# PJLab-ADG/neuralsim

Hardware: NVIDIA H100
Metric: Mrays/sec fwd+bwd (higher is better)
Workload: dtype f16

## Files before the change

### neuralsim_b200/csrc/color_tc.cu

```cuda
#include "fused_tc_common.cuh"
#include "sh_device.cuh"

namespace nsb {

struct ColorNetDev {
    DecoderDevTC dec;
    const __half *R1, *rb1, *R2, *rb2, *R3, *rb3;
    int rw, rin, n_appear;
    float fac[3];
};

constexpr int XW = 64;
constexpr int kTileBytes = kTile * XW * 2;
constexpr int kChunk = kTile * 16;

__host__ __device__ inline int ref_col(int k, int n_appear) {
    if (k < 32) return 22 + k;
    if (k < 35) return k - 32;
    if (k < 51) return 3 + (k - 35);
    if (k < 54) return 19 + (k - 51);
    if (k < 54 + n_appear) return k;
    return -1;
}


__device__ __forceinline__ void level_jacobian(const PLMeta &m, uint32_t p, const float (&xs)[3], const __half *__restrict__ grid,
                                               float (&J0)[3], float (&J1)[3]) {
    uint32_t cell[8];
    float w[8], fr[3], scale[3];
    level_cells3(m, p, xs, cell, w, fr, scale);
    const uint32_t *lp = level_cells_ptr(m, p, grid);
    float2 v[8];
#pragma unroll
    for (int c = 0; c < 8; ++c) {
        const uint32_t raw = ld_nc_u32(lp + cell[c]);
        v[c] = __half22float2(*reinterpret_cast<const __half2 *>(&raw));
    }
#pragma unroll
    for (int gd = 0; gd < 3; ++gd) {
        float a0 = 0.f, a1 = 0.f;
#pragma unroll
        for (int c = 0; c < 4; ++c) {
            float ww = scale[gd];
            int left = 0;
#pragma unroll
            for (int k = 0; k < 2; ++k) {
                const int d = k >= gd ? k + 1 : k;
                if (c & (1 << k)) { ww = __fmul_rn(ww, fr[d]); left += 1 << d; }
                else ww = __fmul_rn(ww, __fsub_rn(1.f, fr[d]));
            }
            const int right = left + (1 << gd);
            a0 = __fmaf_rn(ww, __fsub_rn(v[right].x, v[left].x), a0);
            a1 = __fmaf_rn(ww, __fsub_rn(v[right].y, v[left].y), a1);
        }
        J0[gd] = a0;
        J1[gd] = a1;
    }
}

__device__ __forceinline__ void unpack8(const uint4 &q, float (&v)[8]) {
    const __half2 *h = reinterpret_cast<const __half2 *>(&q);
#pragma unroll
    for (int i = 0; i < 4; ++i) { const float2 f = __half22float2(h[i]); v[2 * i] = f.x; v[2 * i + 1] = f.y; }
}

constexpr int kColorGatherU = 4;

constexpr int kColorBwdCtasPerSM = 2;

__global__ void __launch_bounds__(kTile)
k_color_fwd(const PLMeta m, const __half *__restrict__ grid, const ColorNetDev net, const PointSrc ps, const float *__restrict__ view_dirs,
            const float *__restrict__ h_appear, int64_t n, int max_level, float *__restrict__ sdf_out, float *__restrict__ nab_out,
            float *__restrict__ rgb_out, float *__restrict__ x_out, uint8_t *__restrict__ Zt, uint8_t *__restrict__ Xt,
            uint8_t *__restrict__ Y1t, uint8_t *__restrict__ Y2t, const OccCollect oc, const int64_t *__restrict__ n_dev) {
    n = eff_n(n, n_dev);
    extern __shared__ uint8_t dyn_smem[];
    uint8_t *tiles = reinterpret_cast<uint8_t *>((reinterpret_cast<uintptr_t>(dyn_smem) + 1023) & ~uintptr_t(1023));
    uint8_t *sX = tiles;
    uint8_t *sU = sX + kTileBytes;
    uint8_t *sW1 = sU + kTileBytes;
    uint8_t *sW1T = sW1 + HW * NF * 2;
    uint8_t *sR1 = sW1T + HW * NF * 2;
    uint8_t *sR2 = sR1 + XW * XW * 2;
    constexpr int kS = tc::acc_stride(64);
    float *acc = reinterpret_cast<float *>(sR2 + XW * XW * 2);
    __shared__ float sb1[HW], sW2[HW], srb1[XW], srb2[XW], sR3[3][XW];
    __shared__ float sb2, srb3[3];

    const int tid = threadIdx.x;
    stage_W1(net.dec, sW1, tid);
    stage_W1T(net.dec, sW1T, tid);
    for (int e = tid; e < XW * XW; e += kTile) {
        const int j = e % XW, k = e / XW;
        const int rc = ref_col(k, net.n_appear);
        const __half v1 = (j < net.rw && rc >= 0) ? net.R1[j * net.rin + rc] : __float2half_rn(0.f);
        const __half v2 = (j < net.rw && k < net.rw) ? net.R2[j * net.rw + k] : __float2half_rn(0.f);
        *reinterpret_cast<__half *>(sR1 + (k / 8) * (XW * 16) + j * 16 + (k % 8) * 2) = v1;
        *reinterpret_cast<__half *>(sR2 + (k / 8) * (XW * 16) + j * 16 + (k % 8) * 2) = v2;
    }
    stage_decoder_vectors(net.dec, sb1, sW2, &sb2, tid);
    if (tid < XW) {
        srb1[tid] = tid < net.rw ? __half2float(net.rb1[tid]) : 0.f;
        srb2[tid] = tid < net.rw ? __half2float(net.rb2[tid]) : 0.f;
#pragma unroll
        for (int k = 0; k < 3; ++k) sR3[k][tid] = tid < net.rw ? __half2float(net.R3[k * net.rw + tid]) : 0.f;
    }
    if (tid == 0) {
        for (int k = 0; k < 3; ++k) srb3[k] = __half2float(net.rb3[k]);
    }
    tc::fence_async_smem();
    __syncthreads();
    const uint32_t x_addr = tc::smem_u32(sX), u_addr = tc::smem_u32(sU), w1_addr = tc::smem_u32(sW1), w1t_addr = tc::smem_u32(sW1T);
    const uint32_t r1_addr = tc::smem_u32(sR1), r2_addr = tc::smem_u32(sR2);
    const SoftplusK spk(net.dec.beta);

    const int64_t n_tiles = (n + kTile - 1) / kTile;
    for (int64_t tile = blockIdx.x; tile < n_tiles; tile += gridDim.x) {
        const int64_t i = tile * kTile + tid;
        const bool valid = i < n;
        float xn[3], xs[3];
        int64_t ray;
        load_point(ps, ps.x == nullptr, i, valid, xn, xs, ray);
        gather_row_to_tile<kTile, kColorGatherU>(m, grid, xs, max_level, sX, tid);
        tc::fence_async_smem();
        __syncthreads();
        tc::mma_to_rows<64, 0, 0, NF / 16>(acc, kS, 0, tc::kmajor(x_addr, kTile), tc::kmajor(w1_addr, HW), false);
        __syncthreads();
        float out = 0.f;
        uint8_t *zt = Zt ? Zt + tile * kTileBytes : nullptr;
#pragma unroll 1
        for (int c = 0; c < HW / 8; ++c) {
            float z[8], uu[8];
            tc::acc_ld8(acc, kS, tid, c * 8, z);
#pragma unroll
            for (int j = 0; j < 8; ++j) {
                z[j] = r16(z[j] + sb1[c * 8 + j]);
                float a, s;
                softplus_as(z[j], spk, a, s);
                out = fmaf(r16(a), sW2[c * 8 + j], out);
                uu[j] = sW2[c * 8 + j] * s;
            }
            *reinterpret_cast<uint4 *>(sU + c * kChunk + tid * 16) = tc::pack8_f16(uu);
            if (zt) *reinterpret_cast<uint4 *>(zt + c * kChunk + tid * 16) = tc::pack8_f16(z);
        }
        const float sdf = r16(out + sb2);
        tc::fence_async_smem();
        __syncthreads();
        tc::mma_to_rows<32, 0, 0, HW / 16>(acc, kS, 0, tc::kmajor(u_addr, kTile), tc::kmajor(w1t_addr, NF), false);
        __syncthreads();
        float nacc[3] = {0.f, 0.f, 0.f};
#pragma unroll 1
        for (uint32_t g4 = 0; g4 < 4; ++g4) {
            float gg[8];
            tc::acc_ld8(acc, kS, tid, g4 * 8, gg);
#pragma unroll
            for (uint32_t q = 0; q < 4; ++q) {
                const uint32_t p = g4 * 4 + q;
                if ((int)m.level[p] <= max_level) {
                    float J0[3], J1[3];
                    level_jacobian(m, p, xs, grid, J0, J1);
                    const float g0 = r16(gg[2 * q]), g1 = r16(gg[2 * q + 1]);
#pragma unroll
                    for (int d = 0; d < 3; ++d) nacc[d] = __fmaf_rn(g0, J0[d], nacc[d]);
#pragma unroll
                    for (int d = 0; d < 3; ++d) nacc[d] = __fmaf_rn(g1, J1[d], nacc[d]);
                }
            }
        }
        float nab[3];
#pragma unroll
        for (int d = 0; d < 3; ++d) nab[d] = __fmul_rn(__fmul_rn(nacc[d], 0.5f), net.fac[d]);
        {
            float xr[32];
#pragma unroll
            for (int k = 0; k < 32; ++k) xr[k] = 0.f;
            xr[0] = xn[0]; xr[1] = xn[1]; xr[2] = xn[2];
            if (valid) {
                sh_basis(view_dirs[ray * 3], view_dirs[ray * 3 + 1], view_dirs[ray * 3 + 2], 4, xr + 3);
                if (h_appear) {
#pragma unroll
                    for (int k = 0; k < 8; ++k)
                        if (k < net.n_appear) xr[22 + k] = h_appear[ray * net.n_appear + k];
                }
            }
#pragma unroll
            for (int d = 0; d < 3; ++d) xr[19 + d] = fminf(fmaxf(nab[d], -1.f), 1.f);
            uint8_t *xt = Xt ? Xt + tile * kTileBytes : nullptr;
#pragma unroll
            for (int c = 0; c < 4; ++c) {
                float v8[8];
#pragma unroll
                for (int k = 0; k < 8; ++k) v8[k] = xr[c * 8 + k];
                const uint4 q = tc::pack8_f16(v8);
                *reinterpret_cast<uint4 *>(sX + (4 + c) * kChunk + tid * 16) = q;
                if (xt) {
                    *reinterpret_cast<uint4 *>(xt + (4 + c) * kChunk + tid * 16) = q;
                    *reinterpret_cast<uint4 *>(xt + c * kChunk + tid * 16) = *reinterpret_cast<const uint4 *>(sX + c * kChunk + tid * 16);
                }
            }
        }
        tc::fence_async_smem();
        __syncthreads();
        tc::mma_to_rows<64, 0, 0, XW / 16>(acc, kS, 0, tc::kmajor(x_addr, kTile), tc::kmajor(r1_addr, XW), false);
        __syncthreads();
        uint8_t *y1t = Y1t ? Y1t + tile * kTileBytes : nullptr;
#pragma unroll 1
        for (int c = 0; c < XW / 8; ++c) {
            float y[8];
            tc::acc_ld8(acc, kS, tid, c * 8, y);
#pragma unroll
            for (int j = 0; j < 8; ++j) y[j] = fmaxf(r16(y[j] + srb1[c * 8 + j]), 0.f);
            const uint4 q = tc::pack8_f16(y);
            *reinterpret_cast<uint4 *>(sU + c * kChunk + tid * 16) = q;
            if (y1t) *reinterpret_cast<uint4 *>(y1t + c * kChunk + tid * 16) = q;
        }
        tc::fence_async_smem();
        __syncthreads();
        tc::mma_to_rows<64, 0, 0, XW / 16>(acc, kS, 0, tc::kmajor(u_addr, kTile), tc::kmajor(r2_addr, XW), false);
        __syncthreads();
        float o3[3] = {0.f, 0.f, 0.f};
        uint8_t *y2t = Y2t ? Y2t + tile * kTileBytes : nullptr;
#pragma unroll 1
        for (int c = 0; c < XW / 8; ++c) {
            float y[8];
            tc::acc_ld8(acc, kS, tid, c * 8, y);
#pragma unroll
            for (int j = 0; j < 8; ++j) {
                y[j] = fmaxf(r16(y[j] + srb2[c * 8 + j]), 0.f);
#pragma unroll
                for (int k = 0; k < 3; ++k) o3[k] = fmaf(y[j], sR3[k][c * 8 + j], o3[k]);
            }
            if (y2t) *reinterpret_cast<uint4 *>(y2t + c * kChunk + tid * 16) = tc::pack8_f16(y);
        }
        if (valid) {
            sdf_out[i] = sdf;
            if (oc.pcl) occ_collect_point(oc, xs, sdf);
#pragma unroll
            for (int d = 0; d < 3; ++d) {
                nab_out[i * 3 + d] = nab[d];
                const float y3 = r16(o3[d] + srb3[d]);
                rgb_out[i * 3 + d] = r16(1.f / (1.f + expf(-y3)));
                if (x_out) x_out[i * 3 + d] = xn[d];
            }
        }
        __syncthreads();
    }
}

__global__ void __launch_bounds__(kTile, kColorBwdCtasPerSM)
k_color_rad_bwd(const ColorNetDev net, const uint8_t *__restrict__ Xt, const uint8_t *__restrict__ Y1t, const uint8_t *__restrict__ Y2t,
                const float *__restrict__ rgb, const float *__restrict__ g_rgb, int64_t n, float *__restrict__ dh_out,
                float *__restrict__ dR1, float *__restrict__ drb1, float *__restrict__ dR2, float *__restrict__ drb2,
                float *__restrict__ dR3, float *__restrict__ drb3, const int64_t *__restrict__ n_dev) {
    n = eff_n(n, n_dev);
    constexpr int NE = 80;
    extern __shared__ uint8_t dyn_smem[];
    uint8_t *tiles = reinterpret_cast<uint8_t *>((reinterpret_cast<uintptr_t>(dyn_smem) + 1023) & ~uintptr_t(1023));
    uint8_t *sT = tiles;
    uint8_t *sY1 = sT + 3 * kTileBytes;
    uint8_t *sXe = sY1 + kTile * NE * 2;
    uint8_t *sR2T = sXe + kTile * NE * 2;
    uint8_t *sR1h = sR2T + XW * XW * 2;
    __shared__ float sR3[3][XW];
    __shared__ float sdb3[3];
    __shared__ __align__(8) uint64_t mbar_ld;

    const int tid = threadIdx.x, lane = tid & 31;
    for (int e = tid; e < XW * XW; e += kTile) {
        const int i = e % XW, j = e / XW;
        const __half v = (j < net.rw && i < net.rw) ? net.R2[j * net.rw + i] : __float2half_rn(0.f);
        *reinterpret_cast<__half *>(sR2T + (j / 8) * (XW * 16) + i * 16 + (j % 8) * 2) = v;
    }
    for (int e = tid; e < NF * XW; e += kTile) {
        const int k = e % NF, j = e / NF;
        const __half v = j < net.rw ? net.R1[j * net.rin + 22 + k] : __float2half_rn(0.f);
        *reinterpret_cast<__half *>(sR1h + (j / 8) * (NF * 16) + k * 16 + (j % 8) * 2) = v;
    }
    if (tid < XW) {
#pragma unroll
        for (int k = 0; k < 3; ++k) sR3[k][tid] = tid < net.rw ? __half2float(net.R3[k * net.rw + tid]) : 0.f;
    }
    *reinterpret_cast<uint4 *>(sY1 + 8 * kChunk + tid * 16) = make_uint4(0x00003C00u, 0, 0, 0);
    *reinterpret_cast<uint4 *>(sY1 + 9 * kChunk + tid * 16) = make_uint4(0, 0, 0, 0);
    *reinterpret_cast<uint4 *>(sXe + 9 * kChunk + tid * 16) = make_uint4(0, 0, 0, 0);
    float xa[NE / 2], xb[NE / 2], x3[4];
#pragma unroll
    for (int k = 0; k < NE / 2; ++k) xa[k] = xb[k] = 0.f;
#pragma unroll
    for (int k = 0; k < 4; ++k) x3[k] = 0.f;
    if (tid == 0) {
        sdb3[0] = sdb3[1] = sdb3[2] = 0.f;
        tc::mbar_init(&mbar_ld, 1);
        tc::fence_mbar_init();
    }
    tc::fence_async_smem();
    __syncthreads();
    const uint32_t t_addr = tc::smem_u32(sT), y1_addr = tc::smem_u32(sY1), xe_addr = tc::smem_u32(sXe);
    const uint32_t r2t_addr = tc::smem_u32(sR2T), r1h_addr = tc::smem_u32(sR1h);
    uint32_t ld_phase = 0;
    bool first_tile = true;

    const int64_t n_tiles = (n + kTile - 1) / kTile;
    auto fetch = [&](int64_t tile) {
        tc::mbar_arrive_expect_tx(&mbar_ld, 3 * kTileBytes);
        tc::tma_load_bulk(sT + 2 * kTileBytes, Y2t + tile * kTileBytes, kTileBytes, &mbar_ld);
        tc::tma_load_bulk(sY1, Y1t + tile * kTileBytes, kTileBytes, &mbar_ld);
        tc::tma_load_bulk(sXe, Xt + tile * kTileBytes, kTileBytes, &mbar_ld);
    };
    if (tid == 0 && (int64_t)blockIdx.x < n_tiles) fetch(blockIdx.x);
    for (int64_t tile = blockIdx.x; tile < n_tiles; tile += gridDim.x) {
        const int64_t i = tile * kTile + tid;
        const bool valid = i < n;
        tc::mbar_wait(&mbar_ld, ld_phase);
        ld_phase ^= 1;
        float gy[3] = {0.f, 0.f, 0.f};
        if (valid && g_rgb) {
#pragma unroll
            for (int k = 0; k < 3; ++k) {
                const float y = rgb[i * 3 + k];
                gy[k] = r16(r16(g_rgb[i * 3 + k]) * ((1.f - y) * y));
            }
        }
        {
            float e8[8] = {1.f, gy[0], gy[1], gy[2], 0.f, 0.f, 0.f, 0.f};
            *reinterpret_cast<uint4 *>(sXe + 8 * kChunk + tid * 16) = tc::pack8_f16(e8);
        }
#pragma unroll
        for (int k = 0; k < 3; ++k) {
            const float sgy = warp_sum(gy[k]);
            if (lane == 0 && sgy != 0.f) atomicAdd(&sdb3[k], sgy);
        }
#pragma unroll 1
        for (int c = 0; c < 8; ++c) {
            float y2[8], d[8];
            unpack8(*reinterpret_cast<const uint4 *>(sT + 2 * kTileBytes + c * kChunk + tid * 16), y2);
#pragma unroll
            for (int j = 0; j < 8; ++j) {
                const float v = gy[0] * sR3[0][c * 8 + j] + gy[1] * sR3[1][c * 8 + j] + gy[2] * sR3[2][c * 8 + j];
                d[j] = y2[j] > 0.f ? v : 0.f;
            }
            *reinterpret_cast<uint4 *>(sT + c * kChunk + tid * 16) = tc::pack8_f16(d);
        }
        tc::fence_async_smem();
        __syncthreads();
        {
            float dy[2][XW / 2];
            tc::mma_m128<64, 0, 0, XW / 16>(dy, tc::kmajor(t_addr, kTile), tc::kmajor(r2t_addr, XW), false);
#pragma unroll
            for (int h = 0; h < 2; ++h)
#pragma unroll
                for (int c = 0; c < XW / 8; ++c)
#pragma unroll
                    for (int r = 0; r < 2; ++r) {
                        const uint32_t off = tc::pair_off<kTile>(h * 64 + tc::frag_row(r), tc::frag_col(c));
                        const float2 y1 = tc::ld_pair_f16(sY1, off);
                        tc::st_pair_f16(sT + kTileBytes, off, y1.x > 0.f ? dy[h][4 * c + 2 * r] : 0.f, y1.y > 0.f ? dy[h][4 * c + 2 * r + 1] : 0.f);
                    }
        }
        tc::fence_async_smem();
        __syncthreads();
        float dh[2][NF / 2];
        tc::mma_m128<32, 0, 0, XW / 16>(dh, tc::kmajor(t_addr + kTileBytes, kTile), tc::kmajor(r1h_addr, NF), false);
        tc::mma_m64<NE, 1, 1, kTile / 16>(xa, tc::mnmajor(t_addr, kTile), tc::mnmajor(y1_addr, kTile), true);
        tc::mma_m64<NE, 1, 1, kTile / 16>(xb, tc::mnmajor(t_addr + kTileBytes, kTile), tc::mnmajor(xe_addr, kTile), true);
        tc::mma_m64<8, 1, 1, kTile / 16>(x3, tc::mnmajor(t_addr + 2 * kTileBytes, kTile), tc::mnmajor(xe_addr + 8 * kChunk, kTile), true);
        first_tile = false;
        __syncthreads();
        if (tid == 0 && tile + gridDim.x < n_tiles) {
            tc::fence_async_smem();
            fetch(tile + gridDim.x);
        }
#pragma unroll
        for (int h = 0; h < 2; ++h)
#pragma unroll
            for (int r = 0; r < 2; ++r) {
                const int64_t row = tile * kTile + h * 64 + tc::frag_row(r);
                if (row < n) {
#pragma unroll
                    for (int c = 0; c < NF / 8; ++c)
                        *reinterpret_cast<float2 *>(dh_out + row * NF + tc::frag_col(c)) = make_float2(dh[h][4 * c + 2 * r], dh[h][4 * c + 2 * r + 1]);
                }
            }
    }
    if (!first_tile) {
#pragma unroll
        for (int r = 0; r < 2; ++r) {
            const int row = tc::frag_row(r);
            if (row >= net.rw) continue;
#pragma unroll
            for (int c = 0; c < NE / 8; ++c)
#pragma unroll
                for (int j = 0; j < 2; ++j) {
                    const int col = tc::frag_col(c) + j;
                    const float a = xa[4 * c + 2 * r + j], b = xb[4 * c + 2 * r + j];
                    if (col < XW) {
                        if (col < net.rw) atomicAdd(dR2 + row * net.rw + col, a);
                        const int rc = ref_col(col, net.n_appear);
                        if (rc >= 0) atomicAdd(dR1 + row * net.rin + rc, b);
                    } else if (col == XW) {
                        atomicAdd(drb2 + row, a);
                        atomicAdd(drb1 + row, b);
                    }
                }
#pragma unroll
            for (int j = 0; j < 2; ++j) {
                const int col = tc::frag_col(0) + j;
                if (col >= 1 && col <= 3) atomicAdd(dR3 + (col - 1) * net.rw + row, x3[2 * r + j]);
            }
        }
        if (tid < 3) atomicAdd(drb3 + tid, sdb3[tid]);
    }
}

__global__ void __launch_bounds__(kTile, kColorBwdCtasPerSM)
k_color_sdf_bwd(const PLMeta m, const __half *__restrict__ grid, const ColorNetDev net, const PointSrc ps, const uint8_t *__restrict__ Zt,
                const uint8_t *__restrict__ Xt, const float *__restrict__ g_nab, const float *__restrict__ g_sdf, const float *__restrict__ dh_r,
                int64_t n, int max_level, float *__restrict__ d_grid, float *__restrict__ d_W1, float *__restrict__ d_b1, float *__restrict__ d_W2,
                float *__restrict__ d_b2, const int64_t *__restrict__ n_dev) {
    n = eff_n(n, n_dev);
    constexpr int NX = 48;
    extern __shared__ uint8_t dyn_smem[];
    uint8_t *tiles = reinterpret_cast<uint8_t *>((reinterpret_cast<uintptr_t>(dyn_smem) + 1023) & ~uintptr_t(1023));
    uint8_t *sT = tiles;
    uint8_t *sHe = sT + 3 * kTileBytes;
    uint8_t *sGe = sHe + kTile * NX * 2;
    uint8_t *sW1 = sGe + kTile * NX * 2;
    uint8_t *sW1T = sW1 + HW * NF * 2;
    uint8_t *sZ = sW1T + NF * HW * 2;
    constexpr int kS = tc::acc_stride(2 * NF);
    float *stage = reinterpret_cast<float *>(sT);
    static_assert(kTile * kS * 4 <= 3 * kTileBytes, "the staged rows must fit in T");
    __shared__ float sW2[HW], sdsdf[kTile];
    __shared__ float sdb2;
    __shared__ __align__(8) uint64_t mbar_ld;

    const int tid = threadIdx.x, lane = tid & 31;
    stage_W1(net.dec, sW1, tid);
    stage_W1T(net.dec, sW1T, tid);
    stage_decoder_vectors(net.dec, nullptr, sW2, nullptr, tid);
    *reinterpret_cast<uint4 *>(sHe + 4 * kChunk + tid * 16) = make_uint4(0x00003C00u, 0, 0, 0);
    *reinterpret_cast<uint4 *>(sGe + 4 * kChunk + tid * 16) = make_uint4(0x00003C00u, 0, 0, 0);
    *reinterpret_cast<uint4 *>(sHe + 5 * kChunk + tid * 16) = make_uint4(0, 0, 0, 0);
    *reinterpret_cast<uint4 *>(sGe + 5 * kChunk + tid * 16) = make_uint4(0, 0, 0, 0);
    float wacc[NX / 2], vacc[4];
#pragma unroll
    for (int k = 0; k < NX / 2; ++k) wacc[k] = 0.f;
#pragma unroll
    for (int k = 0; k < 4; ++k) vacc[k] = 0.f;
    if (tid == 0) {
        sdb2 = 0.f;
        tc::mbar_init(&mbar_ld, 1);
        tc::fence_mbar_init();
    }
    tc::fence_async_smem();
    __syncthreads();
    const uint32_t t_addr = tc::smem_u32(sT), he_addr = tc::smem_u32(sHe), ge_addr = tc::smem_u32(sGe), w1_addr = tc::smem_u32(sW1),
                   w1t_addr = tc::smem_u32(sW1T);
    const SoftplusK spk(net.dec.beta);
    uint32_t ld_phase = 0;
    bool first_tile = true;

    const int64_t n_tiles = (n + kTile - 1) / kTile;
    auto fetch = [&](int64_t tile) {
        tc::mbar_arrive_expect_tx(&mbar_ld, kTileBytes + 4 * kChunk);
        tc::tma_load_bulk(sZ, Zt + tile * kTileBytes, kTileBytes, &mbar_ld);
        tc::tma_load_bulk(sHe, Xt + tile * kTileBytes, 4 * kChunk, &mbar_ld);
    };
    if (tid == 0 && (int64_t)blockIdx.x < n_tiles) fetch(blockIdx.x);
    for (int64_t tile = blockIdx.x; tile < n_tiles; tile += gridDim.x) {
        const int64_t i = tile * kTile + tid;
        const bool valid = i < n;
        float xn[3], xs[3];
        int64_t ray;
        load_point(ps, ps.x == nullptr, i, valid, xn, xs, ray);
        float gin[3] = {0.f, 0.f, 0.f};
        if (valid && g_nab) {
#pragma unroll
            for (int d = 0; d < 3; ++d) gin[d] = g_nab[i * 3 + d] * net.fac[d] * 0.5f;
        }
        const float dsdf = (valid && g_sdf) ? g_sdf[i] : 0.f;
        sdsdf[tid] = dsdf;
        tc::mbar_wait(&mbar_ld, ld_phase);
        ld_phase ^= 1;
#pragma unroll 1
        for (int c = 0; c < 8; ++c) {
            float z[8], uu[8];
            unpack8(*reinterpret_cast<const uint4 *>(sZ + c * kChunk + tid * 16), z);
#pragma unroll
            for (int j = 0; j < 8; ++j) {
                float a, s;
                softplus_as(z[j], spk, a, s);
                uu[j] = sW2[c * 8 + j] * s;
            }
            *reinterpret_cast<uint4 *>(sT + kTileBytes + c * kChunk + tid * 16) = tc::pack8_f16(uu);
        }
#pragma unroll 4
        for (uint32_t p = 0; p < 16; ++p) {
            uint32_t packed = 0;
            if ((int)m.level[p] <= max_level) {
                float J0[3], J1[3];
                level_jacobian(m, p, xs, grid, J0, J1);
                float a0 = 0.f, a1 = 0.f;
#pragma unroll
                for (int d = 0; d < 3; ++d) { a0 = __fmaf_rn(gin[d], J0[d], a0); a1 = __fmaf_rn(gin[d], J1[d], a1); }
                const __half2 h = __floats2half2_rn(a0, a1);
                packed = *reinterpret_cast<const uint32_t *>(&h);
            }
            *reinterpret_cast<uint32_t *>(sGe + (p >> 2) * kChunk + tid * 16 + (p & 3) * 4) = packed;
        }
        tc::fence_async_smem();
        __syncthreads();
        float gfr[2][NF / 2];
        {
            float du[2][HW / 2];
            tc::mma_m128<64, 0, 0, NF / 16>(du, tc::kmajor(ge_addr, kTile), tc::kmajor(w1_addr, HW), false);
            tc::mma_m128<32, 0, 0, HW / 16>(gfr, tc::kmajor(t_addr + kTileBytes, kTile), tc::kmajor(w1t_addr, NF), false);
#pragma unroll
            for (int h = 0; h < 2; ++h)
#pragma unroll
                for (int r = 0; r < 2; ++r) {
                    const int row = h * 64 + tc::frag_row(r);
                    const float ds = sdsdf[row];
#pragma unroll
                    for (int c = 0; c < HW / 8; ++c) {
                        const int col = tc::frag_col(c);
                        const uint32_t off = tc::pair_off<kTile>(row, col);
                        const float2 z2 = tc::ld_pair_f16(sZ, off);
                        float dz[2], vv[2];
#pragma unroll
                        for (int j = 0; j < 2; ++j) {
                            const float z = j ? z2.y : z2.x;
                            float a, s;
                            softplus_as(z, spk, a, s);
                            const float w2 = sW2[col + j], d = r16(du[h][4 * c + 2 * r + j]);
                            const float curv = (z * spk.k > spk.thr) ? 0.f : spk.beta * s * (1.f - s);
                            dz[j] = d * w2 * curv + ds * w2 * s;
                            vv[j] = d * s + ds * r16(a);
                        }
                        tc::st_pair_f16(sT, off, dz[0], dz[1]);
                        tc::st_pair_f16(sT + 2 * kTileBytes, off, vv[0], vv[1]);
                    }
                }
        }
        tc::fence_async_smem();
        __syncthreads();
        float dhz[2][NF / 2];
        tc::mma_m128<32, 0, 0, HW / 16>(dhz, tc::kmajor(t_addr, kTile), tc::kmajor(w1t_addr, NF), false);
        tc::mma_m64<NX, 1, 1, kTile / 16>(wacc, tc::mnmajor(t_addr, kTile), tc::mnmajor(he_addr, kTile), true);
        tc::mma_m64<NF, 1, 1, kTile / 16>(*reinterpret_cast<float(*)[NF / 2]>(wacc), tc::mnmajor(t_addr + kTileBytes, kTile), tc::mnmajor(ge_addr, kTile), true);
        tc::mma_m64<8, 1, 1, kTile / 16>(vacc, tc::mnmajor(t_addr + 2 * kTileBytes, kTile), tc::mnmajor(ge_addr + 4 * kChunk, kTile), true);
        first_tile = false;
        const float dsum = warp_sum(dsdf);
        if (lane == 0 && dsum != 0.f) atomicAdd(&sdb2, dsum);
        __syncthreads();
        if (tid == 0 && tile + gridDim.x < n_tiles) {
            tc::fence_async_smem();
            fetch(tile + gridDim.x);
        }
        tc::frag_store<NF>(gfr, stage, kS, 0);
        tc::frag_store<NF>(dhz, stage, kS, NF);
        __syncthreads();
#pragma unroll 1
        for (uint32_t g4 = 0; g4 < 4; ++g4) {
            float gg[8], hz[8];
            tc::acc_ld8(stage, kS, tid, g4 * 8, gg);
            tc::acc_ld8(stage, kS, tid, NF + g4 * 8, hz);
            if (valid && dh_r) {
                const float4 r0 = *reinterpret_cast<const float4 *>(dh_r + i * NF + g4 * 8), r1 = *reinterpret_cast<const float4 *>(dh_r + i * NF + g4 * 8 + 4);
                hz[0] += r0.x; hz[1] += r0.y; hz[2] += r0.z; hz[3] += r0.w; hz[4] += r1.x; hz[5] += r1.y; hz[6] += r1.z; hz[7] += r1.w;
            }
#pragma unroll
            for (uint32_t q = 0; q < 4; ++q) {
                const uint32_t p = g4 * 4 + q;
                if ((int)m.level[p] > max_level) continue;
                uint32_t cell[8];
                float w[8], fr[3], sc[3], ua[8], ub[8];
                level_cells3(m, p, xs, cell, w, fr, sc);
                const float g0 = valid ? r16(gg[2 * q]) : 0.f, g1 = valid ? r16(gg[2 * q + 1]) : 0.f;
                const float h0 = valid ? hz[2 * q] : 0.f, h1 = valid ? hz[2 * q + 1] : 0.f;
#pragma unroll
                for (int c = 0; c < 8; ++c) {
                    float wsum = 0.f;
#pragma unroll
                    for (int gd = 0; gd < 3; ++gd) {
                        float ww = __fmul_rn(sc[gd], gin[gd]);
#pragma unroll
                        for (int d = 0; d < 3; ++d) {
                            if (d == gd) continue;
                            ww = __fmul_rn(ww, (c & (1 << d)) ? fr[d] : __fsub_rn(1.f, fr[d]));
                        }
                        wsum += (c & (1 << gd)) ? ww : -ww;
                    }
                    ua[c] = g0 * wsum + h0 * w[c];
                    ub[c] = g1 * wsum + h1 * w[c];
                }
                bool issue = valid;
                if (level_mergeable(m, p)) issue = warp_merge_updates(cell_key3(m, p, xs), valid, ua, ub, lane);
                if (issue) {
                    float2 *gp = level_grad_ptr(m, p, d_grid);
#pragma unroll
                    for (int c = 0; c < 8; ++c) red_add2(gp + cell[c], ua[c], ub[c]);
                }
            }
        }
        __syncthreads();
    }
    if (!first_tile) {
#pragma unroll
        for (int r = 0; r < 2; ++r) {
            const int row = tc::frag_row(r);
            if (row >= net.dec.width) continue;
#pragma unroll
            for (int c = 0; c <= NF / 8; ++c)
#pragma unroll
                for (int j = 0; j < 2; ++j) {
                    const int col = tc::frag_col(c) + j;
                    if (col < NF) atomicAdd(d_W1 + row * NF + col, wacc[4 * c + 2 * r + j]);
                    else if (col == NF) atomicAdd(d_b1 + row, wacc[4 * c + 2 * r + j]);
                }
            if (tc::frag_col(0) == 0) atomicAdd(d_W2 + row, vacc[2 * r]);
        }
        if (tid == 0) atomicAdd(d_b2, sdb2);
    }
}

}

using namespace nsb;

namespace {
int make_net(const nsb_color_net *c, const nsb_lotd_meta *meta, PLMeta *m, ColorNetDev *d, const char *who) {
    const nsb_sdf_decoder dec{c->W1, c->b1, c->W2, c->b2, c->width, c->beta};
    if (int rc = make_decoder(meta, &dec, m, &d->dec, who)) return rc;
    NSB_REQUIRE(c->rad_width >= 1 && c->rad_width <= 64, "%s: radiance width must be <= 64", who);
    NSB_REQUIRE(c->n_appear >= 0 && c->n_appear <= 8 && c->rad_in == 54 + c->n_appear,
                "%s: radiance input must be [x(3), SH deg 4 (16), n(3), h(32), h_appear(<=8)]", who);
    d->R1 = (const __half *)c->R1; d->rb1 = (const __half *)c->rb1; d->R2 = (const __half *)c->R2; d->rb2 = (const __half *)c->rb2;
    d->R3 = (const __half *)c->R3; d->rb3 = (const __half *)c->rb3;
    d->rw = c->rad_width; d->rin = c->rad_in; d->n_appear = c->n_appear;
    for (int k = 0; k < 3; ++k) d->fac[k] = c->nablas_scale[k];
    return 0;
}
}

static int64_t n_tiles(int64_t n) { return (n + kTile - 1) / kTile; }

extern "C" int64_t nsb_color_tile_bytes(int64_t n) { return n_tiles(n) * (int64_t)kTileBytes; }

extern "C" int nsb_fused_color_fwd(const nsb_lotd_meta *meta, const void *params_half, const nsb_color_net *net, const float *x, const float *rays_o,
                                   const float *rays_d, const int64_t *ridx, const float *t, const float *view_dirs, const float *h_appear,
                                   int64_t n, int32_t max_level, float *sdf, float *nablas, float *rgb, float *x_out, void *act_z, void *act_x,
                                   void *act_y1, void *act_y2, const nsb_occ_collect *collect, void *stream) {
    const DevCounts dn = take_counts();
    if (n == 0) return 0;
    NSB_REQUIRE(meta && params_half && net && sdf && nablas && rgb && view_dirs, "nsb_fused_color_fwd: NULL argument");
    NSB_REQUIRE(x || (rays_o && rays_d && t), "nsb_fused_color_fwd: need x or (rays_o, rays_d, t)");
    NSB_REQUIRE((act_z && act_x && act_y1 && act_y2) || (!act_z && !act_x && !act_y1 && !act_y2), "nsb_fused_color_fwd: pass all four activation buffers or none");
    PLMeta m;
    ColorNetDev d;
    if (int rc = make_net(net, meta, &m, &d, "nsb_fused_color_fwd")) return rc;
    NSB_REQUIRE(d.n_appear == 0 || h_appear, "nsb_fused_color_fwd: h_appear is NULL but the net has %d appearance channels", d.n_appear);
    constexpr int kSmem = 2 * kTileBytes + 2 * HW * NF * 2 + 2 * XW * XW * 2 + kTile * tc::acc_stride(64) * 4 + 1024;
    opt_in_smem(k_color_fwd, kSmem);
    const PointSrc ps{x, rays_o, rays_d, t, ridx};
    k_color_fwd<<<persistent_grid(n_tiles(n), 2), kTile, kSmem, (cudaStream_t)stream>>>(m, (const __half *)params_half, d, ps, view_dirs, h_appear, n,
                                                                                        max_level < 0 ? -1 : max_level, sdf, nablas, rgb, x_out, (uint8_t *)act_z,
                                                                                        (uint8_t *)act_x, (uint8_t *)act_y1, (uint8_t *)act_y2,
                                                                                        occ_collect_of(collect), dn.a);
    return check_launch("nsb_fused_color_fwd");
}

extern "C" int nsb_fused_color_bwd(const nsb_lotd_meta *meta, const void *params_half, const nsb_color_net *net, const float *x, const float *rays_o,
                                   const float *rays_d, const int64_t *ridx, const float *t, int64_t n, int32_t max_level, const void *act_z,
                                   const void *act_x, const void *act_y1, const void *act_y2, const float *rgb, const float *g_sdf,
                                   const float *g_nablas, const float *g_rgb, float *dh_scratch, float *d_grid, float *d_W1, float *d_b1,
                                   float *d_W2, float *d_b2, float *d_R1, float *d_rb1, float *d_R2, float *d_rb2, float *d_R3, float *d_rb3,
                                   void *stream) {
    const DevCounts dn = take_counts();
    if (n == 0) return 0;
    NSB_REQUIRE(meta && params_half && net && act_z && act_x && act_y1 && act_y2 && rgb && dh_scratch, "nsb_fused_color_bwd: NULL argument");
    NSB_REQUIRE(d_grid && d_W1 && d_b1 && d_W2 && d_b2 && d_R1 && d_rb1 && d_R2 && d_rb2 && d_R3 && d_rb3, "nsb_fused_color_bwd: NULL gradient buffer");
    NSB_REQUIRE(x || (rays_o && rays_d && t), "nsb_fused_color_bwd: need x or (rays_o, rays_d, t)");
    PLMeta m;
    ColorNetDev d;
    if (int rc = make_net(net, meta, &m, &d, "nsb_fused_color_bwd")) return rc;
    cudaStream_t s = (cudaStream_t)stream;
    const float *dh = nullptr;
    if (g_rgb) {
        constexpr int kSmemR = 3 * kTileBytes + 2 * kTile * 80 * 2 + XW * XW * 2 + NF * XW * 2 + 1024;
        opt_in_smem(k_color_rad_bwd, kSmemR);
        if (int rc = require_ctas_per_sm(k_color_rad_bwd, kTile, kSmemR, kColorBwdCtasPerSM, "nsb_fused_color_bwd(radiance)")) return rc;
        k_color_rad_bwd<<<persistent_grid(n_tiles(n), kColorBwdCtasPerSM), kTile, kSmemR, s>>>(d, (const uint8_t *)act_x, (const uint8_t *)act_y1,
                                                                                               (const uint8_t *)act_y2, rgb, g_rgb, n, dh_scratch, d_R1,
                                                                                               d_rb1, d_R2, d_rb2, d_R3, d_rb3, dn.a);
        if (int rc = check_launch("nsb_fused_color_bwd(radiance)")) return rc;
        dh = dh_scratch;
    }
    constexpr int kSmemS = 3 * kTileBytes + 2 * kTile * 48 * 2 + 2 * HW * NF * 2 + kTileBytes + 1024;
    opt_in_smem(k_color_sdf_bwd, kSmemS);
    if (int rc = require_ctas_per_sm(k_color_sdf_bwd, kTile, kSmemS, kColorBwdCtasPerSM, "nsb_fused_color_bwd(sdf)")) return rc;
    const PointSrc ps{x, rays_o, rays_d, t, ridx};
    k_color_sdf_bwd<<<persistent_grid(n_tiles(n), kColorBwdCtasPerSM), kTile, kSmemS, s>>>(m, (const __half *)params_half, d, ps, (const uint8_t *)act_z, (const uint8_t *)act_x,
                                                                          g_nablas, g_sdf, dh, n, max_level < 0 ? -1 : max_level, d_grid, d_W1, d_b1, d_W2, d_b2, dn.a);
    return check_launch("nsb_fused_color_bwd(sdf)");
}
```

### neuralsim_b200/csrc/tc_util.cuh

```cuda
#pragma once
#include "nsb_common.cuh"

namespace nsb {
namespace tc {

__device__ __forceinline__ uint32_t smem_u32(const void *p) { return (uint32_t)__cvta_generic_to_shared(p); }

__device__ __forceinline__ uint64_t make_desc(uint32_t smem_addr, uint32_t lbo_bytes, uint32_t sbo_bytes) {
    uint64_t d = 0;
    d |= (uint64_t)((smem_addr >> 4) & 0x3FFF);
    d |= (uint64_t)((lbo_bytes >> 4) & 0x3FFF) << 16;
    d |= (uint64_t)((sbo_bytes >> 4) & 0x3FFF) << 32;
    return d;
}

struct Operand {
    uint32_t addr, lbo, sbo, kstep;
};
__device__ __forceinline__ Operand kmajor(uint32_t addr, int rows) { return Operand{addr, (uint32_t)rows * 16, 128, (uint32_t)rows * 32}; }
__device__ __forceinline__ Operand mnmajor(uint32_t addr, int rows) { return Operand{addr, 128, (uint32_t)rows * 16, 256}; }

template <int N, int TA, int TB>
struct Wgmma;
template <int TA, int TB>
struct Wgmma<8, TA, TB> {
    __device__ __forceinline__ static void mma(float (&d)[4], uint64_t a, uint64_t b, uint32_t acc) {
        asm volatile(
            "{\n\t.reg .pred p;\n\tsetp.ne.b32 p, %6, 0;\n\t"
            "wgmma.mma_async.sync.aligned.m64n8k16.f32.f16.f16 {%0, %1, %2, %3}, %4, %5, p, 1, 1, %7, %8;\n\t}\n"
            : "+f"(d[0]), "+f"(d[1]), "+f"(d[2]), "+f"(d[3])
            : "l"(a), "l"(b), "r"(acc), "n"(TA), "n"(TB));
    }
};
template <int TA, int TB>
struct Wgmma<32, TA, TB> {
    __device__ __forceinline__ static void mma(float (&d)[16], uint64_t a, uint64_t b, uint32_t acc) {
        asm volatile(
            "{\n\t.reg .pred p;\n\tsetp.ne.b32 p, %18, 0;\n\t"
            "wgmma.mma_async.sync.aligned.m64n32k16.f32.f16.f16 {%0, %1, %2, %3, %4, %5, %6, %7, %8, %9, %10, %11, %12, %13, %14, %15}, %16, %17, p, 1, 1, %19, %20;\n\t}\n"
            : "+f"(d[0]), "+f"(d[1]), "+f"(d[2]), "+f"(d[3]), "+f"(d[4]), "+f"(d[5]), "+f"(d[6]), "+f"(d[7]), "+f"(d[8]), "+f"(d[9]), "+f"(d[10]), "+f"(d[11]), "+f"(d[12]), "+f"(d[13]), "+f"(d[14]), "+f"(d[15])
            : "l"(a), "l"(b), "r"(acc), "n"(TA), "n"(TB));
    }
};
template <int TA, int TB>
struct Wgmma<40, TA, TB> {
    __device__ __forceinline__ static void mma(float (&d)[20], uint64_t a, uint64_t b, uint32_t acc) {
        asm volatile(
            "{\n\t.reg .pred p;\n\tsetp.ne.b32 p, %22, 0;\n\t"
            "wgmma.mma_async.sync.aligned.m64n40k16.f32.f16.f16 {%0, %1, %2, %3, %4, %5, %6, %7, %8, %9, %10, %11, %12, %13, %14, %15, %16, %17, %18, %19}, %20, %21, p, 1, 1, %23, %24;\n\t}\n"
            : "+f"(d[0]), "+f"(d[1]), "+f"(d[2]), "+f"(d[3]), "+f"(d[4]), "+f"(d[5]), "+f"(d[6]), "+f"(d[7]), "+f"(d[8]), "+f"(d[9]), "+f"(d[10]), "+f"(d[11]), "+f"(d[12]), "+f"(d[13]), "+f"(d[14]), "+f"(d[15]), "+f"(d[16]), "+f"(d[17]), "+f"(d[18]), "+f"(d[19])
            : "l"(a), "l"(b), "r"(acc), "n"(TA), "n"(TB));
    }
};
template <int TA, int TB>
struct Wgmma<48, TA, TB> {
    __device__ __forceinline__ static void mma(float (&d)[24], uint64_t a, uint64_t b, uint32_t acc) {
        asm volatile(
            "{\n\t.reg .pred p;\n\tsetp.ne.b32 p, %26, 0;\n\t"
            "wgmma.mma_async.sync.aligned.m64n48k16.f32.f16.f16 {%0, %1, %2, %3, %4, %5, %6, %7, %8, %9, %10, %11, %12, %13, %14, %15, %16, %17, %18, %19, %20, %21, %22, %23}, %24, %25, p, 1, 1, %27, %28;\n\t}\n"
            : "+f"(d[0]), "+f"(d[1]), "+f"(d[2]), "+f"(d[3]), "+f"(d[4]), "+f"(d[5]), "+f"(d[6]), "+f"(d[7]), "+f"(d[8]), "+f"(d[9]), "+f"(d[10]), "+f"(d[11]), "+f"(d[12]), "+f"(d[13]), "+f"(d[14]), "+f"(d[15]), "+f"(d[16]), "+f"(d[17]), "+f"(d[18]), "+f"(d[19]), "+f"(d[20]), "+f"(d[21]), "+f"(d[22]), "+f"(d[23])
            : "l"(a), "l"(b), "r"(acc), "n"(TA), "n"(TB));
    }
};
template <int TA, int TB>
struct Wgmma<64, TA, TB> {
    __device__ __forceinline__ static void mma(float (&d)[32], uint64_t a, uint64_t b, uint32_t acc) {
        asm volatile(
            "{\n\t.reg .pred p;\n\tsetp.ne.b32 p, %34, 0;\n\t"
            "wgmma.mma_async.sync.aligned.m64n64k16.f32.f16.f16 {%0, %1, %2, %3, %4, %5, %6, %7, %8, %9, %10, %11, %12, %13, %14, %15, %16, %17, %18, %19, %20, %21, %22, %23, %24, %25, %26, %27, %28, %29, %30, %31}, %32, %33, p, 1, 1, %35, %36;\n\t}\n"
            : "+f"(d[0]), "+f"(d[1]), "+f"(d[2]), "+f"(d[3]), "+f"(d[4]), "+f"(d[5]), "+f"(d[6]), "+f"(d[7]), "+f"(d[8]), "+f"(d[9]), "+f"(d[10]), "+f"(d[11]), "+f"(d[12]), "+f"(d[13]), "+f"(d[14]), "+f"(d[15]), "+f"(d[16]), "+f"(d[17]), "+f"(d[18]), "+f"(d[19]), "+f"(d[20]), "+f"(d[21]), "+f"(d[22]), "+f"(d[23]), "+f"(d[24]), "+f"(d[25]), "+f"(d[26]), "+f"(d[27]), "+f"(d[28]), "+f"(d[29]), "+f"(d[30]), "+f"(d[31])
            : "l"(a), "l"(b), "r"(acc), "n"(TA), "n"(TB));
    }
};
template <int TA, int TB>
struct Wgmma<80, TA, TB> {
    __device__ __forceinline__ static void mma(float (&d)[40], uint64_t a, uint64_t b, uint32_t acc) {
        asm volatile(
            "{\n\t.reg .pred p;\n\tsetp.ne.b32 p, %42, 0;\n\t"
            "wgmma.mma_async.sync.aligned.m64n80k16.f32.f16.f16 {%0, %1, %2, %3, %4, %5, %6, %7, %8, %9, %10, %11, %12, %13, %14, %15, %16, %17, %18, %19, %20, %21, %22, %23, %24, %25, %26, %27, %28, %29, %30, %31, %32, %33, %34, %35, %36, %37, %38, %39}, %40, %41, p, 1, 1, %43, %44;\n\t}\n"
            : "+f"(d[0]), "+f"(d[1]), "+f"(d[2]), "+f"(d[3]), "+f"(d[4]), "+f"(d[5]), "+f"(d[6]), "+f"(d[7]), "+f"(d[8]), "+f"(d[9]), "+f"(d[10]), "+f"(d[11]), "+f"(d[12]), "+f"(d[13]), "+f"(d[14]), "+f"(d[15]), "+f"(d[16]), "+f"(d[17]), "+f"(d[18]), "+f"(d[19]), "+f"(d[20]), "+f"(d[21]), "+f"(d[22]), "+f"(d[23]), "+f"(d[24]), "+f"(d[25]), "+f"(d[26]), "+f"(d[27]), "+f"(d[28]), "+f"(d[29]), "+f"(d[30]), "+f"(d[31]), "+f"(d[32]), "+f"(d[33]), "+f"(d[34]), "+f"(d[35]), "+f"(d[36]), "+f"(d[37]), "+f"(d[38]), "+f"(d[39])
            : "l"(a), "l"(b), "r"(acc), "n"(TA), "n"(TB));
    }
};

__device__ __forceinline__ void wgmma_fence() { asm volatile("wgmma.fence.sync.aligned;" ::: "memory"); }
__device__ __forceinline__ void wgmma_commit() { asm volatile("wgmma.commit_group.sync.aligned;" ::: "memory"); }
__device__ __forceinline__ void wgmma_wait_all() { asm volatile("wgmma.wait_group.sync.aligned 0;" ::: "memory"); }
__device__ __forceinline__ void fence_operand(float &r) { asm volatile("" : "+f"(r)::"memory"); }

template <int N, int TA, int TB, int KSTEPS>
__device__ __forceinline__ void mma_m128(float (&d)[2][N / 2], const Operand &a, const Operand &b, bool accumulate) {
#pragma unroll
    for (int h = 0; h < 2; ++h)
#pragma unroll
        for (int i = 0; i < N / 2; ++i) fence_operand(d[h][i]);
    wgmma_fence();
#pragma unroll
    for (int h = 0; h < 2; ++h)
#pragma unroll
        for (int ks = 0; ks < KSTEPS; ++ks)
            Wgmma<N, TA, TB>::mma(d[h], make_desc(a.addr + h * 8 * a.sbo + ks * a.kstep, a.lbo, a.sbo), make_desc(b.addr + ks * b.kstep, b.lbo, b.sbo),
                                  (ks > 0 || accumulate) ? 1u : 0u);
    wgmma_commit();
    wgmma_wait_all();
#pragma unroll
    for (int h = 0; h < 2; ++h)
#pragma unroll
        for (int i = 0; i < N / 2; ++i) fence_operand(d[h][i]);
}

template <int N, int TA, int TB, int KSTEPS>
__device__ __forceinline__ void mma_m64(float (&d)[N / 2], const Operand &a, const Operand &b, bool accumulate) {
#pragma unroll
    for (int i = 0; i < N / 2; ++i) fence_operand(d[i]);
    wgmma_fence();
#pragma unroll
    for (int ks = 0; ks < KSTEPS; ++ks)
        Wgmma<N, TA, TB>::mma(d, make_desc(a.addr + ks * a.kstep, a.lbo, a.sbo), make_desc(b.addr + ks * b.kstep, b.lbo, b.sbo),
                              (ks > 0 || accumulate) ? 1u : 0u);
    wgmma_commit();
    wgmma_wait_all();
#pragma unroll
    for (int i = 0; i < N / 2; ++i) fence_operand(d[i]);
}

__device__ __forceinline__ int frag_row(int i) { return (threadIdx.x >> 5) * 16 + ((threadIdx.x & 31) >> 2) + 8 * i; }
__device__ __forceinline__ int frag_col(int c) { return c * 8 + 2 * (threadIdx.x & 3); }
template <int R>
__device__ __forceinline__ uint32_t pair_off(int row, int col) { return (uint32_t)((col >> 3) * (R * 16) + row * 16 + (col & 7) * 2); }
__device__ __forceinline__ float2 ld_pair_f16(const uint8_t *tile, uint32_t off) {
    return __half22float2(*reinterpret_cast<const __half2 *>(tile + off));
}
__device__ __forceinline__ void st_pair_f16(uint8_t *tile, uint32_t off, float a, float b) {
    *reinterpret_cast<__half2 *>(tile + off) = __floats2half2_rn(a, b);
}

constexpr int acc_stride(int cols) { return cols + 4; }

template <int N>
__device__ __forceinline__ void frag_store(const float (&d)[2][N / 2], float *acc, int stride, int col0) {
    const int w = threadIdx.x >> 5, l = threadIdx.x & 31;
#pragma unroll
    for (int h = 0; h < 2; ++h)
#pragma unroll
        for (int c = 0; c < N / 8; ++c)
#pragma unroll
            for (int i = 0; i < 2; ++i) {
                const int row = h * 64 + w * 16 + (l >> 2) + 8 * i, col = col0 + c * 8 + 2 * (l & 3);
                *reinterpret_cast<float2 *>(acc + row * stride + col) = make_float2(d[h][4 * c + 2 * i], d[h][4 * c + 2 * i + 1]);
            }
}
template <int N>
__device__ __forceinline__ void frag_load(float (&d)[2][N / 2], const float *acc, int stride, int col0) {
    const int w = threadIdx.x >> 5, l = threadIdx.x & 31;
#pragma unroll
    for (int h = 0; h < 2; ++h)
#pragma unroll
        for (int c = 0; c < N / 8; ++c)
#pragma unroll
            for (int i = 0; i < 2; ++i) {
                const int row = h * 64 + w * 16 + (l >> 2) + 8 * i, col = col0 + c * 8 + 2 * (l & 3);
                const float2 v = *reinterpret_cast<const float2 *>(acc + row * stride + col);
                d[h][4 * c + 2 * i] = v.x;
                d[h][4 * c + 2 * i + 1] = v.y;
            }
}
template <int N, int TA, int TB, int KSTEPS>
__device__ __forceinline__ void mma_to_rows(float *acc, int stride, int col0, const Operand &a, const Operand &b, bool accumulate) {
    float d[2][N / 2];
    if (accumulate) frag_load<N>(d, acc, stride, col0);
    else {
#pragma unroll
        for (int h = 0; h < 2; ++h)
#pragma unroll
            for (int i = 0; i < N / 2; ++i) d[h][i] = 0.f;
    }
    mma_m128<N, TA, TB, KSTEPS>(d, a, b, accumulate);
    frag_store<N>(d, acc, stride, col0);
}

__device__ __forceinline__ void acc_ld8(const float *acc, int stride, int row, int col, float (&v)[8]) {
    const float4 a = *reinterpret_cast<const float4 *>(acc + row * stride + col), b = *reinterpret_cast<const float4 *>(acc + row * stride + col + 4);
    v[0] = a.x; v[1] = a.y; v[2] = a.z; v[3] = a.w; v[4] = b.x; v[5] = b.y; v[6] = b.z; v[7] = b.w;
}

__device__ __forceinline__ void mbar_init(uint64_t *bar, uint32_t count) {
    asm volatile("mbarrier.init.shared::cta.b64 [%0], %1;" ::"r"(smem_u32(bar)), "r"(count) : "memory");
}
__device__ __forceinline__ void mbar_wait(uint64_t *bar, uint32_t parity) {
    asm volatile(
        "{\n\t.reg .pred p;\n\tWAIT_%=:\n\t"
        "mbarrier.try_wait.parity.shared::cta.b64 p, [%0], %1;\n\t"
        "@p bra DONE_%=;\n\tbra WAIT_%=;\n\tDONE_%=:\n\t}\n" ::"r"(smem_u32(bar)),
        "r"(parity)
        : "memory");
}

__device__ __forceinline__ void mbar_arrive_expect_tx(uint64_t *bar, uint32_t bytes) {
    asm volatile("mbarrier.arrive.expect_tx.shared::cta.b64 _, [%0], %1;" ::"r"(smem_u32(bar)), "r"(bytes) : "memory");
}
__device__ __forceinline__ void tma_load_bulk(void *smem_dst, const void *gmem_src, uint32_t bytes, uint64_t *bar) {
    asm volatile("cp.async.bulk.shared::cluster.global.mbarrier::complete_tx::bytes [%0], [%1], %2, [%3];" ::"r"(smem_u32(smem_dst)), "l"(gmem_src),
                 "r"(bytes), "r"(smem_u32(bar))
                 : "memory");
}

__device__ __forceinline__ void fence_async_smem() { asm volatile("fence.proxy.async.shared::cta;" ::: "memory"); }
__device__ __forceinline__ void fence_mbar_init() { asm volatile("fence.mbarrier_init.release.cluster;" ::: "memory"); }

__device__ __forceinline__ uint4 pack8_f16(const float (&v)[8]) {
    __half2 h0 = __floats2half2_rn(v[0], v[1]), h1 = __floats2half2_rn(v[2], v[3]);
    __half2 h2 = __floats2half2_rn(v[4], v[5]), h3 = __floats2half2_rn(v[6], v[7]);
    uint4 q;
    q.x = *reinterpret_cast<uint32_t *>(&h0); q.y = *reinterpret_cast<uint32_t *>(&h1);
    q.z = *reinterpret_cast<uint32_t *>(&h2); q.w = *reinterpret_cast<uint32_t *>(&h3);
    return q;
}

template <int R, int K>
__device__ __forceinline__ void store_row_f16(uint8_t *tile, int r, const float *vals) {
#pragma unroll
    for (int c = 0; c < K / 8; ++c) {
        __half2 h0 = __floats2half2_rn(vals[c * 8 + 0], vals[c * 8 + 1]);
        __half2 h1 = __floats2half2_rn(vals[c * 8 + 2], vals[c * 8 + 3]);
        __half2 h2 = __floats2half2_rn(vals[c * 8 + 4], vals[c * 8 + 5]);
        __half2 h3 = __floats2half2_rn(vals[c * 8 + 6], vals[c * 8 + 7]);
        uint4 q;
        q.x = *reinterpret_cast<uint32_t *>(&h0);
        q.y = *reinterpret_cast<uint32_t *>(&h1);
        q.z = *reinterpret_cast<uint32_t *>(&h2);
        q.w = *reinterpret_cast<uint32_t *>(&h3);
        *reinterpret_cast<uint4 *>(tile + c * (R * 16) + r * 16) = q;
    }
}

}
}
```

### neuralsim_b200/fields/fused_color.py

```python
from __future__ import annotations

import ctypes

import torch
from torch import autograd

from .. import _lib as L


class _FusedColor(autograd.Function):
    @staticmethod
    def forward(ctx, model, pts, view_dirs, h_appear, max_level, keep, collect, *params):
        grid16, net, _held = model._fused_color_state()
        ridx, t, rays_o, rays_d = pts
        n, dev = t.numel(), t.device
        meta = model.implicit_surface.encoding.meta
        sdf = torch.empty(n, dtype=torch.float32, device=dev)
        nab = torch.empty(n, 3, dtype=torch.float32, device=dev)
        rgb = torch.empty(n, 3, dtype=torch.float32, device=dev)
        x = torch.empty(n, 3, dtype=torch.float32, device=dev)
        acts = None
        if keep:
            acts = torch.empty(4, int(L.lib().nsb_color_tile_bytes(L.c_i64(n))), dtype=torch.uint8, device=dev)
        ap = [L.ptr(acts[k]) if keep else None for k in range(4)]
        with L.KERNEL_TIMER.time("fused_color_fwd", n):
            L.check(L.lib().nsb_fused_color_fwd(meta.c_ref, L.ptr(grid16, "f16"), ctypes.byref(net), None, L.ptr(rays_o, "f32"), L.ptr(rays_d, "f32"),
                                                L.ptr(ridx, "i64"), L.ptr(t, "f32"), L.ptr(view_dirs, "f32"), L.ptr(h_appear, "f32", allow_none=True),
                                                L.c_i64(n), L.c_i32(max_level), L.ptr(sdf), L.ptr(nab), L.ptr(rgb), L.ptr(x), *ap,
                                                ctypes.byref(collect) if collect is not None else None, L.stream_ptr()),
                    "fused_color_fwd")
        ctx.model, ctx.pts, ctx.max_level, ctx.n = model, pts, max_level, n
        ctx.held = (grid16, net, _held, acts, rgb)
        ctx.shapes = [p.shape for p in params]
        ctx.set_materialize_grads(False)
        ctx.mark_non_differentiable(x)
        return sdf, nab, rgb, x

    @staticmethod
    @autograd.function.once_differentiable
    def backward(ctx, g_sdf, g_nab, g_rgb, _gx):
        grid16, net, _held, acts, rgb = ctx.held
        if acts is None:
            raise RuntimeError("fused_color: backward through a forward that ran without grad")
        dev, n = rgb.device, ctx.n
        meta = ctx.model.implicit_surface.encoding.meta
        sizes = [int(torch.Size(s).numel()) for s in ctx.shapes[1:]]
        small = torch.zeros(sum(sizes), dtype=torch.float32, device=dev)
        grads, o = [torch.zeros(ctx.shapes[0], dtype=torch.float32, device=dev)], 0
        for sh, k in zip(ctx.shapes[1:], sizes):
            grads.append(small[o:o + k].view(sh))
            o += k
        if g_sdf is None and g_nab is None and g_rgb is None:
            return (None,) * 7 + tuple(grads)
        ridx, t, rays_o, rays_d = ctx.pts
        c = lambda g: None if g is None else g.contiguous().float()
        g_sdf, g_nab, g_rgb = c(g_sdf), c(g_nab), c(g_rgb)
        dh = torch.empty(n, 32, dtype=torch.float32, device=dev)
        with L.KERNEL_TIMER.time("fused_color_bwd", n):
            L.check(L.lib().nsb_fused_color_bwd(meta.c_ref, L.ptr(grid16, "f16"), ctypes.byref(net), None, L.ptr(rays_o, "f32"), L.ptr(rays_d, "f32"),
                                                L.ptr(ridx, "i64"), L.ptr(t, "f32"), L.c_i64(n), L.c_i32(ctx.max_level), L.ptr(acts[0]), L.ptr(acts[1]),
                                                L.ptr(acts[2]), L.ptr(acts[3]), L.ptr(rgb), L.ptr(g_sdf, allow_none=True), L.ptr(g_nab, allow_none=True),
                                                L.ptr(g_rgb, allow_none=True), L.ptr(dh), *[L.ptr(g) for g in grads], L.stream_ptr()),
                    "fused_color_bwd")
        return (None,) * 7 + tuple(grads)


def fused_color(model, ridx, t, rays_o, rays_d, view_dirs, h_appear=None, *, nablas_has_grad=True, collect=None):
    s, r = model.implicit_surface, model.radiance_net.blocks.layers
    d = s.decoder.layers
    params = (s.encoding.flattened_params, d[0].weight, d[0].bias, d[1].weight, d[1].bias, r[0].weight, r[0].bias, r[1].weight, r[1].bias,
              r[2].weight, r[2].bias)
    pts = (ridx.reshape(-1).contiguous().long(), t.detach().reshape(-1).contiguous().float(), rays_o.detach().contiguous().float(),
           rays_d.detach().contiguous().float())
    keep = torch.is_grad_enabled() and any(p.requires_grad for p in params)
    ha = None if h_appear is None else h_appear.detach().contiguous().float()
    sdf, nab, rgb, x = _FusedColor.apply(model, pts, view_dirs.detach().contiguous().float(), ha, s._ml(model.max_level), keep, collect, *params)
    if not nablas_has_grad:
        nab = nab.detach()
    return dict(sdf=sdf, nablas=nab, rgb=rgb, x=x)
```

### neuralsim_b200/graphics/neus_static.py

```python
from __future__ import annotations

import ctypes

import torch
import torch.nn.functional as F

from .. import _lib as L
from .raysample import batch_sample_step_linear
from .pack_ops import get_pack_infos_from_batch
from . import neus_fused as NF

__all__ = ["render_static", "StaticFrame", "CNT_SLOTS"]

CNT_SLOTS = dict(n_rays=0, pairs=2, marched_raw=3, hit_raw=4, kept_raw=6, kept_rays_raw=7, nonzero=9, marched=12, hit=13, fine0=14,
                 boundary=18, kept=19, overflow=20, kept_rays=21, merged0=22, rays_if_kept_fits=26)
_NULL = ctypes.c_void_p(0)
MARCH_ONEPASS = "auto"
MARCH_ONEPASS_MAX_BYTES = 64 << 20


def march_onepass(n_rays, max_steps):
    if MARCH_ONEPASS == "0":
        return False
    return MARCH_ONEPASS == "1" or 4 * int(n_rays) * int(max_steps) <= MARCH_ONEPASS_MAX_BYTES


def _slot(cnt, k):
    return ctypes.c_void_p(cnt.data_ptr() + 8 * k)


def _call(fn, what, cnt, k0, k1, *args):
    lib = L.lib()
    lib.nsb_bind_device_counts(_slot(cnt, k0), _slot(cnt, k1) if k1 is not None else _NULL)
    try:
        rc = fn(*args)
    finally:
        lib.nsb_bind_device_counts(_NULL, _NULL)
    L.check(rc, what)


def _scan(counts, cnt, slot, *, first=None, info2=None, index=None, pack=None, src=None, nz_src=None, ws=None):
    if ws is None:
        ws = torch.zeros(NF._scan_ws_bytes(), dtype=torch.uint8, device=counts.device)
    P = L.ptr
    L.check(L.lib().nsb_scan_counts(P(counts, "i32"), L.c_i64(counts.shape[0]), P(first, allow_none=True), P(info2, allow_none=True),
                                    P(index, allow_none=True), P(pack, allow_none=True), P(src, "i64", allow_none=True), P(nz_src, allow_none=True),
                                    _slot(cnt, slot), None, L.c_i64(0), P(ws), L.stream_ptr()), "scan_counts")


def _query_counts(cnt, phase, n_coarse1, num_fine, march_cap, kept_cap):
    nf = (ctypes.c_int32 * max(len(num_fine), 1))(*[int(n) for n in num_fine])
    L.check(L.lib().nsb_query_counts(ctypes.c_void_p(cnt.data_ptr()), L.c_i32(phase), L.c_i32(n_coarse1), nf, L.c_i32(len(num_fine)),
                                     L.c_i64(march_cap), L.c_i64(kept_cap), L.stream_ptr()), "query_counts")


def _sdf_launch(meta, grid16, dec, rays_o, rays_d, t, sdf, *, ridx=None, packs=None, ml, collect, cnt, slot, timer="lotd_gather"):
    P = L.ptr
    mode = 2 if packs is not None else 1
    with L.KERNEL_TIMER.time(timer, t.numel()):
        _call(L.lib().nsb_fused_sdf_collect, "fused_sdf", cnt, slot, None,
              meta.c_ref, P(grid16, "f16"), ctypes.byref(dec), None, P(rays_o, "f32"), P(rays_d, "f32"),
              P(ridx, "i64") if mode == 1 else None, P(t, "f32"), L.c_i64(t.numel()),
              P(packs[0], "i64") if mode == 2 else None, P(packs[1], "i64", allow_none=True) if mode == 2 else None,
              L.c_i64(packs[0].shape[0] if mode == 2 else 0), L.c_i32(mode), L.c_i32(ml), P(sdf),
              ctypes.byref(collect) if collect is not None else None, L.stream_ptr())
    return sdf


class _StaticSDF(torch.autograd.Function):

    @staticmethod
    def forward(ctx, st, ridx, t, packs, count_slot, grid, W1, b1, W2, b2):
        sdf = torch.empty(t.numel(), dtype=torch.float32, device=t.device)
        _sdf_launch(st.meta, st.grid16, st.dec, st.rays_o, st.rays_d, t, sdf, ridx=ridx if packs is None else None, packs=packs, ml=st.ml,
                    collect=st.collect, cnt=st.cnt, slot=count_slot, timer="fused_sdf_fwd")
        ctx.st, ctx.ridx, ctx.t = st, ridx, t
        ctx.shapes = (grid.shape, W1.shape, b1.shape, W2.shape, b2.shape)
        return sdf

    @staticmethod
    @torch.autograd.function.once_differentiable
    def backward(ctx, d_sdf):
        st, dev = ctx.st, d_sdf.device
        gs, w1s, b1s, w2s, b2s = ctx.shapes
        d_grid = torch.zeros(gs, dtype=torch.float32, device=dev)
        ks = [int(torch.Size(x).numel()) for x in (w1s, b1s, w2s, b2s)]
        small = torch.zeros(sum(ks), dtype=torch.float32, device=dev)
        d_W1, d_b1 = small[:ks[0]].view(w1s), small[ks[0]:ks[0] + ks[1]].view(b1s)
        d_W2, d_b2 = small[ks[0] + ks[1]:ks[0] + ks[1] + ks[2]].view(w2s), small[ks[0] + ks[1] + ks[2]:].view(b2s)
        d_sdf = d_sdf.contiguous().float()
        n = d_sdf.numel()
        P, cnt = L.ptr, st.cnt
        flag = torch.empty(n, dtype=torch.int32, device=dev)
        _call(L.lib().nsb_flag_nonzero, "flag_nonzero", cnt, CNT_SLOTS["boundary"], None, P(d_sdf, "f32"), L.c_i64(n), P(flag), L.stream_ptr())
        keep = torch.empty(n, dtype=torch.int64, device=dev)
        _scan(flag, cnt, CNT_SLOTS["nonzero"], index=keep, ws=st.ws[3])
        with L.KERNEL_TIMER.time("fused_sdf_bwd", n):
            _call(L.lib().nsb_fused_sdf_bwd_indexed, "fused_sdf_bwd", cnt, CNT_SLOTS["nonzero"], None,
                  st.meta.c_ref, P(st.grid16, "f16"), ctypes.byref(st.dec), None, P(st.rays_o, "f32"), P(st.rays_d, "f32"), P(ctx.ridx, "i64"),
                  P(ctx.t, "f32"), P(d_sdf, "f32"), P(keep, "i64"), L.c_i64(n), L.c_i32(st.ml), P(d_grid), P(d_W1), P(d_b1), P(d_W2), P(d_b2),
                  L.stream_ptr())
        return None, None, None, None, None, d_grid, d_W1, d_b1, d_W2, d_b2


class _StaticAlpha(torch.autograd.Function):

    @staticmethod
    def forward(ctx, sdf, inv_s, pack_infos, cnt, early_stop_eps, alpha_thre):
        sdf_c, inv_c = sdf.detach().contiguous().float(), inv_s.detach().contiguous().float().reshape(1)
        Pn, dev = pack_infos.shape[0], sdf_c.device
        alpha = torch.empty_like(sdf_c)
        sel = torch.empty(sdf_c.shape[0], dtype=torch.bool, device=dev)
        steps = torch.empty(Pn, dtype=torch.int32, device=dev)
        P = L.ptr
        _call(L.lib().nsb_neus_alpha_forward, "neus_alpha_forward", cnt, CNT_SLOTS["n_rays"], None, P(sdf_c, "f32"), P(pack_infos, "i64"), L.c_i64(Pn),
              P(inv_c, "f32"), L.c_f32(early_stop_eps), L.c_f32(alpha_thre), P(alpha), P(sel), P(steps), L.stream_ptr())
        ctx.save_for_backward(sdf_c, inv_c, pack_infos)
        ctx.cnt, ctx.inv_shape = cnt, inv_s.shape
        ctx.mark_non_differentiable(sel, steps)
        return alpha, sel, steps

    @staticmethod
    def backward(ctx, g_alpha, _gs, _gn):
        sdf_c, inv_c, pack_infos = ctx.saved_tensors
        g = g_alpha.contiguous().float()
        d_sdf = torch.empty_like(sdf_c)
        d_inv = torch.zeros(1, device=sdf_c.device, dtype=torch.float32)
        P = L.ptr
        _call(L.lib().nsb_neus_alpha_backward, "neus_alpha_backward", ctx.cnt, CNT_SLOTS["n_rays"], None, P(sdf_c, "f32"), P(pack_infos, "i64"),
              L.c_i64(pack_infos.shape[0]), P(inv_c, "f32"), P(g, "f32"), P(d_sdf), P(d_inv), L.stream_ptr())
        return (d_sdf if ctx.needs_input_grad[0] else None, d_inv.reshape(ctx.inv_shape) if ctx.needs_input_grad[1] else None, None, None, None, None)


class _StaticGather(torch.autograd.Function):

    @staticmethod
    def forward(ctx, src, pidx, gathered, cnt):
        ctx.save_for_backward(pidx)
        ctx.n, ctx.cnt = src.shape[0], cnt
        return gathered

    @staticmethod
    def backward(ctx, g):
        pidx, = ctx.saved_tensors
        g = g.contiguous().float()
        d = torch.zeros(ctx.n, dtype=torch.float32, device=g.device)
        P = L.ptr
        _call(L.lib().nsb_scatter_f32, "scatter_f32", ctx.cnt, CNT_SLOTS["kept"], None, P(g, "f32"), P(pidx, "i64"), L.c_i64(pidx.shape[0]), P(d), L.stream_ptr())
        return d, None, None, None


class _StaticColor(torch.autograd.Function):

    @staticmethod
    def forward(ctx, st, ridx, t, view_dirs, h_appear, keep_acts, *params):
        n, dev = t.numel(), t.device
        sdf = torch.empty(n, dtype=torch.float32, device=dev)
        nab = torch.empty(n, 3, dtype=torch.float32, device=dev)
        rgb = torch.empty(n, 3, dtype=torch.float32, device=dev)
        x = torch.empty(n, 3, dtype=torch.float32, device=dev)
        acts = torch.empty(4, int(L.lib().nsb_color_tile_bytes(L.c_i64(n))), dtype=torch.uint8, device=dev) if keep_acts else None
        ap = [L.ptr(acts[k]) if keep_acts else None for k in range(4)]
        P = L.ptr
        with L.KERNEL_TIMER.time("fused_color_fwd", n):
            _call(L.lib().nsb_fused_color_fwd, "fused_color_fwd", st.cnt, CNT_SLOTS["kept"], None,
                  st.meta.c_ref, P(st.grid16, "f16"), ctypes.byref(st.net), None, P(st.rays_o, "f32"), P(st.rays_d, "f32"), P(ridx, "i64"), P(t, "f32"),
                  P(view_dirs, "f32"), P(h_appear, "f32", allow_none=True), L.c_i64(n), L.c_i32(st.ml), P(sdf), P(nab), P(rgb), P(x), *ap,
                  ctypes.byref(st.collect) if st.collect is not None else None, L.stream_ptr())
        ctx.st, ctx.ridx, ctx.t, ctx.n = st, ridx, t, n
        ctx.held = (acts, rgb)
        ctx.shapes = [p.shape for p in params]
        ctx.set_materialize_grads(False)
        ctx.mark_non_differentiable(x)
        return sdf, nab, rgb, x

    @staticmethod
    @torch.autograd.function.once_differentiable
    def backward(ctx, g_sdf, g_nab, g_rgb, _gx):
        acts, rgb = ctx.held
        if acts is None:
            raise RuntimeError("static colour query: backward through a forward that ran without grad")
        st, dev, n = ctx.st, rgb.device, ctx.n
        sizes = [int(torch.Size(s).numel()) for s in ctx.shapes[1:]]
        small = torch.zeros(sum(sizes), dtype=torch.float32, device=dev)
        grads, o = [torch.zeros(ctx.shapes[0], dtype=torch.float32, device=dev)], 0
        for sh, k in zip(ctx.shapes[1:], sizes):
            grads.append(small[o:o + k].view(sh))
            o += k
        if g_sdf is None and g_nab is None and g_rgb is None:
            return (None,) * 6 + tuple(grads)
        c = lambda g: None if g is None else g.contiguous().float()
        g_sdf, g_nab, g_rgb = c(g_sdf), c(g_nab), c(g_rgb)
        dh = torch.empty(n, 32, dtype=torch.float32, device=dev)
        P = L.ptr
        with L.KERNEL_TIMER.time("fused_color_bwd", n):
            _call(L.lib().nsb_fused_color_bwd, "fused_color_bwd", st.cnt, CNT_SLOTS["kept"], None,
                  st.meta.c_ref, P(st.grid16, "f16"), ctypes.byref(st.net), None, P(st.rays_o, "f32"), P(st.rays_d, "f32"), P(ctx.ridx, "i64"),
                  P(ctx.t, "f32"), L.c_i64(n), L.c_i32(st.ml), P(acts[0]), P(acts[1]), P(acts[2]), P(acts[3]), P(rgb), P(g_sdf, allow_none=True),
                  P(g_nab, allow_none=True), P(g_rgb, allow_none=True), P(dh), *[P(g) for g in grads], L.stream_ptr())
        return (None,) * 6 + tuple(grads)


class _StaticComposite(torch.autograd.Function):

    @staticmethod
    def forward(ctx, alpha, t, rgb, nablas, pack_infos, ray_index, n_rays, cnt, normalize_depth, early_stop_eps, alpha_thre):
        a, tt = alpha.detach().contiguous().float(), t.detach().contiguous().float()
        r = None if rgb is None else rgb.detach().contiguous().float()
        nb = None if nablas is None else nablas.detach().contiguous().float()
        Pn, dev = pack_infos.shape[0], a.device
        vw = torch.empty_like(a)
        cols = 2 + (3 if r is not None else 0) + (3 if nb is not None else 0)
        buf = torch.zeros(cols * n_rays, device=dev)
        mask, depth = buf[:n_rays], buf[n_rays:2 * n_rays]
        rgb_o = buf[2 * n_rays:5 * n_rays].view(n_rays, 3) if r is not None else None
        o3 = 5 * n_rays if r is not None else 2 * n_rays
        nab_o = buf[o3:o3 + 3 * n_rays].view(n_rays, 3) if nb is not None else None
        P = L.ptr
        _call(L.lib().nsb_composite_forward, "composite_forward", cnt, CNT_SLOTS["kept_rays"], None, P(a, "f32"), P(tt, "f32"), P(r, "f32", allow_none=True),
              P(nb, "f32", allow_none=True), P(pack_infos, "i64"), L.c_i64(Pn), L.c_f32(early_stop_eps), L.c_f32(alpha_thre),
              ctypes.c_int(1 if normalize_depth else 0), P(ray_index, "i64"), P(vw), P(mask), P(depth), P(rgb_o, allow_none=True),
              P(nab_o, allow_none=True), L.stream_ptr())
        ctx.save_for_backward(a, tt, r, nb, vw, pack_infos, mask, depth, ray_index)
        ctx.cfg = (normalize_depth, early_stop_eps, alpha_thre, cnt)
        ctx.set_materialize_grads(False)
        empty = a.new_empty(0)
        return vw, mask, depth, (rgb_o if rgb_o is not None else empty), (nab_o if nab_o is not None else empty)

    @staticmethod
    def backward(ctx, g_vw, g_mask, g_depth, g_rgb, g_nab):
        a, tt, r, nb, vw, pack_infos, mask, depth, ray_index = ctx.saved_tensors
        normalize_depth, eps, thre, cnt = ctx.cfg

        def opt(g, present=True):
            return None if (g is None or not present) else g.contiguous().float()
        g_vw, g_mask, g_depth = opt(g_vw), opt(g_mask), opt(g_depth)
        g_rgb, g_nab = opt(g_rgb, r is not None), opt(g_nab, nb is not None)
        d_alpha = torch.empty_like(a)
        d_rgb = torch.empty_like(r) if r is not None else None
        d_nab = torch.empty_like(nb) if nb is not None else None
        P = L.ptr
        _call(L.lib().nsb_composite_backward, "composite_backward", cnt, CNT_SLOTS["kept_rays"], None,
              P(a, "f32"), P(tt, "f32"), P(r, allow_none=True), P(nb, allow_none=True), P(vw, "f32"), P(pack_infos, "i64"), L.c_i64(pack_infos.shape[0]),
              L.c_f32(eps), L.c_f32(thre), ctypes.c_int(1 if normalize_depth else 0), P(mask), P(depth), P(g_mask, allow_none=True),
              P(g_depth, allow_none=True), P(g_rgb, allow_none=True), P(g_nab, allow_none=True), P(g_vw, allow_none=True), P(ray_index, "i64"),
              P(d_alpha), P(d_rgb, allow_none=True), P(d_nab, allow_none=True), L.stream_ptr())
        return (d_alpha, None, d_rgb, d_nab) + (None,) * 7


class _State:
    __slots__ = ("meta", "grid16", "dec", "net", "held", "rays_o", "rays_d", "ml", "collect", "cnt", "ws")


def _fp16_images(model):
    s, b = model.implicit_surface, model.radiance_net.blocks.layers
    d = s.decoder.layers
    ps = [s.encoding.flattened_params, d[0].weight, d[0].bias, d[1].weight, d[1].bias, b[0].weight, b[0].bias, b[1].weight, b[1].bias, b[2].weight, b[2].bias]
    t = [torch.empty(p.shape, dtype=torch.half, device=p.device) for p in ps]
    with torch.no_grad():
        t[0].copy_(ps[0].detach())
        torch._foreach_copy_(t[1:], [p.detach() for p in ps[1:]])
    dec = L.SdfDecoderC(t[1].data_ptr(), t[2].data_ptr(), t[3].data_ptr(), t[4].data_ptr(), d[0].out_features, float(d[0].activation.beta))
    r3 = s.radius3d_original
    fk = (r3.data_ptr(), r3._version, float(s.sdf_scale))
    if getattr(model, "_fac_cache", (None,))[0] != fk:
        model._fac_cache = (fk, (s.sdf_scale / r3).float().tolist())
    net = L.ColorNetC(*[x.data_ptr() for x in t[1:]], d[0].out_features, b[0].out_features, b[0].in_features, b[0].in_features - 54,
                      float(d[0].activation.beta), (ctypes.c_float * 3)(*model._fac_cache[1]))
    return t, dec, net, ps


def static_supported(model, cfg):
    qp = dict(model.ray_query_cfg.get("query_param", {}) or {})
    occ = getattr(getattr(model, "accel", None), "occ", None)
    return (getattr(model, "_color_fusable", lambda: False)() and model.use_view_dirs and occ is not None and occ.occ_grid.dim() == 3
            and occ.occ_grid.numel() * 4 // 32 <= 96 * 1024 and qp.get("num_coarse", 0) > 0 and len(qp.get("upsample_inv_s_factors", (1, 4, 16))) <= 4
            and qp.get("coarse_step_cfg", {}).get("step_mode", "linear") == "linear" and (cfg.get("with_rgb", True) or cfg.get("with_normal", True)))


def render_static(model, rays_o, rays_d, rays_h_appear=None, *, near=None, far=None, march_cap, kept_cap, coherent=False, with_rgb=True, with_normal=True,
                  perturb=False, training=None, depth_use_normalized_vw=True, cnt=None):
    P, lib = L.ptr, L.lib()
    if perturb:
        raise RuntimeError("render_static: perturb=True is not built (random streams of capacity-sized draws differ from the reference's); "
                           "use the host-sized path (SingleVolumeRenderer.render)")
    training = model.training if training is None else training
    R, dev = rays_o.shape[0], rays_o.device
    qp = dict(model.ray_query_cfg.get("query_param", {}) or {})
    nc1 = int(qp["num_coarse"]) + 1
    factors = list(qp.get("upsample_inv_s_factors", (1, 4, 16)))
    n_stage = len(factors)
    num_fine = qp.get("num_fine", 8)
    num_fine = [num_fine] * n_stage if isinstance(num_fine, int) else list(num_fine)
    num_fine = [n // 2 * 2 + 1 for n in num_fine]
    nf_tot = int(sum(num_fine))
    upsample_inv_s = qp.get("upsample_inv_s", 64.) / model.upsample_s_divisor
    use_est = bool(qp.get("upsample_use_estimate_alpha", False))
    nablas_has_grad = bool(qp.get("nablas_has_grad", False))
    mc = dict(qp.get("march_cfg", {}))
    fac = mc.pop("step_size_factor", 1.0)
    step_size, dt_gamma = mc.get("step_size", 1e-3) * fac, mc.get("dt_gamma", 0.0) * fac
    max_steps, max_step_size = int(mc.get("max_steps", 512)), mc.get("max_step_size", 1e10)
    march_cap, kept_cap = int(march_cap), int(kept_cap)
    S_cap = R * (nc1 + nf_tot)
    if cnt is None:
        cnt = torch.zeros(32, dtype=torch.int64, device=dev)
    else:
        cnt.zero_()
    st = _State()
    st.cnt = cnt
    wsb = (NF._scan_ws_bytes() + 255) // 256 * 256
    st.ws = torch.zeros(4, wsb, dtype=torch.uint8, device=dev)
    with torch.no_grad():
        t16, st.dec, st.net, masters = _fp16_images(model)
        st.held, st.grid16 = t16, t16[0]
        st.meta = model.implicit_surface.encoding.meta
        st.ml = model.implicit_surface._ml(model.max_level)
        st.collect = model.accel.occ.collect_struct() if training else None
        sp = model.space
        if getattr(sp, "_host_cr", None) is None or sp._host_cr[0] != (sp.aabb.data_ptr(), sp.aabb._version):
            c, r = sp.center.tolist(), sp.radius3d.tolist()
            sp._host_cr = ((sp.aabb.data_ptr(), sp.aabb._version), (ctypes.c_float * 3)(*c), (ctypes.c_float * 3)(*r))
        o_n, d_n = torch.empty(R, 3, device=dev), torch.empty(R, 3, device=dev)
        nr, fr = torch.empty(R, device=dev), torch.empty(R, device=dev)
        flag = torch.empty(R, dtype=torch.int32, device=dev)
        L.check(lib.nsb_ray_test_aabb(P(rays_o.contiguous(), "f32"), P(rays_d.contiguous(), "f32"), L.c_i64(R), sp._host_cr[1], sp._host_cr[2],
                                      ctypes.c_int(0 if near is None else 1), L.c_f32(0. if near is None else near),
                                      ctypes.c_int(0 if far is None else 1), L.c_f32(0. if far is None else far), P(o_n), P(d_n), P(nr), P(fr), P(flag),
                                      _slot(cnt, CNT_SLOTS["pairs"]), L.stream_ptr()), "ray_test_aabb")
        rays_inds = torch.empty(R, dtype=torch.int64, device=dev)
        _scan(flag, cnt, CNT_SLOTS["n_rays"], index=rays_inds, ws=st.ws[0])
        ha = rays_h_appear.detach().contiguous().float() if (rays_h_appear is not None and model.use_h_appear) else None
        if ha is None and model.use_h_appear:
            ha = torch.zeros(R, model.radiance_net.blocks.layers[0].in_features - 54, device=dev)
        n_ha = ha.shape[1] if ha is not None else 0
        rbuf = torch.zeros(R * (8 + n_ha), device=dev)
        o_c, d_c = rbuf[:3 * R].view(R, 3), rbuf[3 * R:6 * R].view(R, 3)
        n_c, f_c = rbuf[6 * R:7 * R], rbuf[7 * R:8 * R]
        ha_c = rbuf[8 * R:].view(R, n_ha) if ha is not None else None
        _call(lib.nsb_gather_rays, "gather_rays", cnt, CNT_SLOTS["n_rays"], None, P(rays_inds, "i64"), L.c_i64(R), P(o_n), P(d_n), P(nr), P(fr), P(o_c), P(d_c),
              P(n_c), P(f_c), P(ha, allow_none=True), P(ha_c, allow_none=True), L.c_i32(0 if ha is None else ha.shape[1]), L.stream_ptr())
        st.rays_o, st.rays_d = o_c, d_c
        view_dirs = (d_c / d_c.norm(dim=-1).clamp_min(1.0e-10).unsqueeze(-1)).contiguous()
        coarse = batch_sample_step_linear(n_c, f_c, nc1, prefix_shape=[R], perturb=perturb).contiguous()
        occ_grid = model.accel.occ.occ_grid
        res = occ_grid.shape[-3:]
        g8 = occ_grid.contiguous().view(torch.uint8)
        bits = torch.empty((occ_grid.numel() + 31) // 32, dtype=torch.int32, device=dev)
        L.check(lib.nsb_pack_occ_bits(P(g8, "u8"), L.c_i64(occ_grid.numel()), P(bits), L.stream_ptr()), "pack_occ_bits")
        roi = torch.tensor([-1, -1, -1, 1, 1, 1], dtype=torch.float32, device=dev) if getattr(model, "_static_roi", None) is None else model._static_roi
        model._static_roi = roi
        margs = (L.c_i64(R), P(o_c, "f32"), P(d_c, "f32"), P(n_c, "f32"), P(f_c, "f32"), P(roi, "f32"), None, L.c_i32(res[0]), L.c_i32(res[1]), L.c_i32(res[2]),
                 P(g8, "u8"), L.c_f32(step_size), L.c_f32(max_step_size), L.c_f32(dt_gamma), ctypes.c_uint32(max_steps))
        num_steps = torch.empty(R, dtype=torch.int32, device=dev)
        rec_t = torch.empty(R * max_steps, dtype=torch.float32, device=dev) if march_onepass(R, max_steps) else None
        with L.KERNEL_TIMER.time("march", R):
            if rec_t is not None:
                _call(lib.nsb_ray_marching_record, "ray_marching_record", cnt, CNT_SLOTS["n_rays"], None, L.c_i64(R), P(o_c, "f32"), P(d_c, "f32"), P(n_c, "f32"),
                      P(f_c, "f32"), P(roi, "f32"), L.c_i32(res[0]), L.c_i32(res[1]), L.c_i32(res[2]), P(g8, "u8"), L.c_f32(step_size), L.c_f32(max_step_size),
                      L.c_f32(dt_gamma), ctypes.c_uint32(max_steps), P(num_steps), P(rec_t), P(bits), L.stream_ptr())
            else:
                _call(lib.nsb_ray_marching_listed, "ray_marching", cnt, CNT_SLOTS["n_rays"], None, *margs, None, P(num_steps), None, None, None, None, None, None,
                      L.c_i64(0), P(bits), L.stream_ptr())
        info2 = torch.empty(R, 2, dtype=torch.int32, device=dev)
        ridx_hit = torch.empty(R, dtype=torch.int64, device=dev)
        pack_infos = torch.empty(R, 2, dtype=torch.int64, device=dev)
        _scan(num_steps, cnt, CNT_SLOTS["marched_raw"], info2=info2, index=ridx_hit, pack=pack_infos, ws=st.ws[1])
        _query_counts(cnt, 0, nc1, num_fine, march_cap, kept_cap)
        depth = torch.empty(march_cap, dtype=torch.float32, device=dev)
        ridx32 = torch.empty(march_cap, dtype=torch.int32, device=dev)
        with L.KERNEL_TIMER.time("march", R):
            if rec_t is not None:
                _call(lib.nsb_march_compact, "march_compact", cnt, CNT_SLOTS["hit"], None, P(rec_t, "f32"), ctypes.c_uint32(max_steps), P(info2, "i32"),
                      P(ridx_hit, "i64"), L.c_i64(R), P(depth), P(ridx32), L.stream_ptr())
            else:
                _call(lib.nsb_ray_marching_listed, "ray_marching", cnt, CNT_SLOTS["hit"], None, *margs, P(info2), None, P(depth), None, P(ridx32), None, None,
                      P(ridx_hit, "i64"), L.c_i64(R), P(bits), L.stream_ptr())
        ridx = ridx32.long()
        from . import neus as GN
        fine_stages = None
        if GN.use_persistent_upsample(R):
            fine_all, _ovf = NF.upsample_rays(st.meta, st.grid16, st.dec, ridx_hit, pack_infos, depth, o_c, d_c, [upsample_inv_s * f for f in factors], num_fine,
                                              max_level=st.ml, max_steps=max_steps, use_estimate_alpha=use_est, collect=st.collect, count=(cnt, CNT_SLOTS["hit"]))
            factors_loop = []
        else:
            factors_loop = factors
        sdf = torch.empty(march_cap if factors_loop else 1, dtype=torch.float32, device=dev)
        if factors_loop:
            fine_stages = []
            _sdf_launch(st.meta, st.grid16, st.dec, o_c, d_c, depth, sdf, ridx=ridx, ml=st.ml, collect=st.collect, cnt=cnt, slot=CNT_SLOTS["marched"])
        for i, factor in enumerate(factors_loop):
            cdf = torch.empty(march_cap, dtype=torch.float32, device=dev)
            _call(lib.nsb_neus_upsample_cdf, "neus_upsample_cdf", cnt, CNT_SLOTS["hit"], None, P(sdf, "f32"), P(depth, "f32"), P(pack_infos, "i64"), L.c_i64(R),
                  L.c_f32(upsample_inv_s * factor), ctypes.c_int(1 if use_est else 0), L.c_f32(1e-4), L.c_f32(0.0), P(cdf), L.stream_ptr())
            nf = num_fine[i]
            fine = torch.empty(R, nf, dtype=torch.float32, device=dev)
            u = NF._U_CACHE.get((nf, dev))
            if u is None:
                u = NF._U_CACHE[(nf, dev)] = torch.linspace(0., 1., nf + 2, device=dev, dtype=torch.float32)[1:-1].contiguous()
            _call(lib.nsb_packed_invert_cdf_shared_u, "packed_invert_cdf_shared_u", cnt, CNT_SLOTS["hit"], None, P(depth, "f32"), P(cdf, "f32"), P(u, "f32"),
                  P(pack_infos, "i64"), L.c_i64(R), L.c_i32(nf), P(fine), L.stream_ptr())
            fine_stages.append(fine)
            if i < n_stage - 1:
                sdf_fine = torch.empty(R * nf, dtype=torch.float32, device=dev)
                if coherent:
                    _sdf_launch(st.meta, st.grid16, st.dec, o_c, d_c, fine.view(-1), sdf_fine, packs=(get_pack_infos_from_batch(R, nf, device=dev), ridx_hit),
                                ml=st.ml, collect=st.collect, cnt=cnt, slot=CNT_SLOTS["hit"])
                else:
                    _sdf_launch(st.meta, st.grid16, st.dec, o_c, d_c, fine.view(-1), sdf_fine, ridx=ridx_hit.unsqueeze(-1).expand(R, nf).reshape(-1).contiguous(),
                                ml=st.ml, collect=st.collect, cnt=cnt, slot=CNT_SLOTS["fine0"] + i)
                dep_m = torch.empty(march_cap, dtype=torch.float32, device=dev)
                sdf_m = torch.empty(march_cap, dtype=torch.float32, device=dev)
                pim = torch.empty_like(pack_infos)
                _call(lib.nsb_merge_sorted_vals, "merge_sorted_vals", cnt, CNT_SLOTS["hit"], None, P(depth, "f32"), P(sdf, "f32"), P(pack_infos, "i64"),
                      P(fine, "f32"), P(sdf_fine, "f32"), L.c_i64(R), L.c_i32(nf), P(dep_m), P(sdf_m), P(pim), L.stream_ptr())
                depth, sdf, pack_infos = dep_m, sdf_m, pim
        if fine_stages is not None:
            fine_all = (torch.cat(fine_stages, dim=-1) if n_stage > 1 else fine_stages[0]).contiguous()
        d1 = torch.empty(S_cap, dtype=torch.float32, device=dev)
        mid = torch.empty(S_cap, dtype=torch.float32, device=dev)
        ridx_all = torch.empty(S_cap, dtype=torch.int64, device=dev)
        pinfo = torch.empty(R, 2, dtype=torch.int64, device=dev)
        rl = (ctypes.c_int32 * n_stage)(*num_fine)
        _call(lib.nsb_assemble_boundary, "assemble_boundary", cnt, CNT_SLOTS["n_rays"], CNT_SLOTS["hit"], P(coarse, "f32"), L.c_i64(R), L.c_i32(nc1),
              P(ridx_hit, "i64"), L.c_i64(R), P(fine_all, "f32"), L.c_i32(nf_tot), rl, L.c_i32(n_stage), P(d1), P(mid), P(ridx_all), P(pinfo), L.stream_ptr())
    s, b = model.implicit_surface, model.radiance_net.blocks.layers
    dl = s.decoder.layers
    sdf_b = _StaticSDF.apply(st, ridx_all, d1, (pinfo, None) if coherent else None, CNT_SLOTS["n_rays"] if coherent else CNT_SLOTS["boundary"],
                             s.encoding.flattened_params, dl[0].weight, dl[0].bias, dl[1].weight, dl[1].bias)
    inv_s = model.forward_inv_s()
    if not isinstance(inv_s, torch.Tensor):
        inv_s = torch.tensor(float(inv_s), device=dev)
    alpha, sel, steps = _StaticAlpha.apply(sdf_b, inv_s, pinfo, cnt, 1e-4, 0.0)
    with torch.no_grad():
        first = torch.empty(R, dtype=torch.int32, device=dev)
        nidx = torch.empty(R, dtype=torch.int64, device=dev)
        pinfo_kept = torch.empty(R, 2, dtype=torch.int64, device=dev)
        rays_inds_hit = torch.empty(R, dtype=torch.int64, device=dev)
        _scan(steps, cnt, CNT_SLOTS["kept_raw"], first=first, index=nidx, pack=pinfo_kept, src=rays_inds, nz_src=rays_inds_hit, ws=st.ws[2])
        _query_counts(cnt, 1, nc1, num_fine, march_cap, kept_cap)
        pidx, ridx_k = torch.empty(kept_cap, dtype=torch.int64, device=dev), torch.empty(kept_cap, dtype=torch.int64, device=dev)
        t_k, alpha_c = torch.empty(kept_cap, dtype=torch.float32, device=dev), torch.empty(kept_cap, dtype=torch.float32, device=dev)
        _call(lib.nsb_compact_samples, "compact_samples", cnt, CNT_SLOTS["rays_if_kept_fits"], None, P(sel.view(torch.uint8), "u8"), P(pinfo, "i64"), P(first, "i32"),
              P(steps, "i32"), L.c_i64(R), P(ridx_all, "i64"), P(mid, "f32"), P(alpha.detach(), "f32"), P(pidx), P(ridx_k), P(t_k), P(alpha_c), L.stream_ptr())
    alpha_k = _StaticGather.apply(alpha, pidx, alpha_c, cnt) if alpha.requires_grad else alpha_c
    params = (s.encoding.flattened_params, dl[0].weight, dl[0].bias, dl[1].weight, dl[1].bias, b[0].weight, b[0].bias, b[1].weight, b[1].bias,
              b[2].weight, b[2].bias)
    keep_acts = torch.is_grad_enabled() and any(p.requires_grad for p in params)
    _sdf_k, nab, rgb, x = _StaticColor.apply(st, ridx_k, t_k, view_dirs, ha_c, keep_acts, *params)
    if not nablas_has_grad:
        nab = nab.detach()
    nab_i = nab if with_normal else None
    if nab_i is not None and not training:
        nab_i = F.normalize(nab_i.clamp(-1, 1), dim=-1)
    vw, m, d, c, nn_ = _StaticComposite.apply(alpha_k, t_k, rgb if with_rgb else None, nab_i, pinfo_kept, rays_inds_hit, R, cnt,
                                              bool(depth_use_normalized_vw), 1e-4, 0.0)
    rendered = dict(mask_volume=m, depth_volume=d)
    if with_rgb:
        rendered["rgb_volume"] = c
    if with_normal:
        rendered["normals_volume"] = nn_
    buffers = dict(opacity_alpha=alpha_k, t=t_k, rgb=rgb, nablas=nab, net_x=x, vw=vw, pack_infos_hit=pinfo_kept, rays_inds_hit=rays_inds_hit, ridx=ridx_k,
                   pack_infos_boundary=pinfo, march_pack_infos=pack_infos)
    return rendered, cnt, buffers


def sliced_volume_buffer(buffers, cnt):
    c = cnt.tolist()
    K, Pu = c[CNT_SLOTS["kept"]], c[CNT_SLOTS["kept_rays"]]
    if c[CNT_SLOTS["overflow"]]:
        raise RuntimeError(f"static step: arena overflow (flags {c[CNT_SLOTS['overflow']]}: 1 = marched samples, 2 = kept samples)")
    if K == 0:
        return dict(type="empty", rays_inds_hit=[])
    vb = dict(type="packed", rays_inds_hit=buffers["rays_inds_hit"][:Pu], pack_infos_hit=buffers["pack_infos_hit"][:Pu])
    for k in ("opacity_alpha", "t", "rgb", "nablas", "net_x", "vw"):
        vb[k] = buffers[k][:K]
    return vb


class StaticFrame:

    def __init__(self, model, n_rays, loss_fn=None, *, near=None, far=None, with_rgb=True, with_normal=True, slack=1.5, march_cap=None, kept_cap=None,
                 coherent=None, use_graph=True, zero_grads=False, h_appear_dim=None, pre_hook=None):
        self.model, self.n_rays, self.loss_fn = model, int(n_rays), loss_fn
        self.near, self.far, self.with_rgb, self.with_normal, self.slack = near, far, with_rgb, with_normal, float(slack)
        self.march_cap, self.kept_cap, self.coherent = march_cap, kept_cap, coherent
        self.use_graph, self.zero_grads, self.pre_hook = use_graph, zero_grads, pre_hook
        dev = model.device
        self.device = dev
        self.rays_o = torch.zeros(self.n_rays, 3, device=dev)
        self.rays_d = torch.zeros(self.n_rays, 3, device=dev)
        na = h_appear_dim if h_appear_dim is not None else (model.radiance_net.blocks.layers[0].in_features - 54 if model.use_h_appear else 0)
        self.h_appear = torch.zeros(self.n_rays, na, device=dev) if na > 0 else None
        self.cnt = torch.zeros(32, dtype=torch.int64, device=dev)
        self.graph, self.loss, self.rendered, self.buffers, self._occ_captured = None, None, None, None, None
        self.captures = 0

    @torch.no_grad()
    def _probe(self):
        from ..renderer import SingleVolumeRenderer
        r = SingleVolumeRenderer(dict(near=self.near, far=self.far, with_rgb=self.with_rgb, with_normal=self.with_normal))
        r.train(self.model.training)
        out = r.ray_query(self.model, self.rays_o, self.rays_d, self.h_appear, return_buffer=True, return_details=True)
        det, vb = out.get("details", {}), out["volume_buffer"]
        qp = dict(self.model.ray_query_cfg.get("query_param", {}) or {})
        nf = qp.get("num_fine", 8)
        nf = [nf] * len(qp.get("upsample_inv_s_factors", (1, 4, 16))) if isinstance(nf, int) else list(nf)
        nf = [n // 2 * 2 + 1 for n in nf]
        M = int(det["march.num_per_ray"].sum()) if "march.num_per_ray" in det else 0
        n_hit = int(det["march.num_per_ray"].shape[0]) if "march.num_per_ray" in det else 0
        K = int(vb["t"].shape[0]) if vb.get("type") == "packed" else 0
        return M + n_hit * sum(nf[:-1]), K, bool(out["ray_tested"].get("rays_coherent", False))

    def _size(self, grow=1.0):
        need_m, need_k, coh = self._probe()
        if self.coherent is None:
            self.coherent = coh
        floor = 4096 + 8 * min(self.n_rays, 65536)
        m = int(max(need_m * self.slack, floor) * grow)
        k = int(max(need_k * self.slack, floor) * grow)
        self.march_cap = max(self.march_cap or 0, m)
        self.kept_cap = max(self.kept_cap or 0, k)

    def _run(self):
        if self.pre_hook is not None:
            self.pre_hook()
        if self.zero_grads:
            for p in self.model.parameters():
                if p.grad is not None:
                    p.grad.zero_()
        cv = getattr(self.model, "ctrl_var", None)
        if cv is not None and hasattr(cv, "mix_weight"):
            if getattr(cv, "_w_dev", None) is None:
                cv._w_dev = torch.zeros((), device=self.device)
            cv._use_w_dev = True
        try:
            rendered, _, buffers = render_static(self.model, self.rays_o, self.rays_d, self.h_appear, near=self.near, far=self.far, march_cap=self.march_cap,
                                                 kept_cap=self.kept_cap, coherent=bool(self.coherent), with_rgb=self.with_rgb, with_normal=self.with_normal, cnt=self.cnt)
        finally:
            if cv is not None:
                cv._use_w_dev = False
        loss = None
        if self.loss_fn is not None:
            loss = self.loss_fn(rendered)
            if loss.requires_grad:
                loss.backward()
            loss = loss.detach()
        return rendered, buffers, loss

    def capture(self):
        if self.march_cap is None or self.kept_cap is None or self.coherent is None:
            self._size()
        if not self.use_graph:
            self.graph = None
            return self
        if not bool(self.rays_d.any()):
            raise RuntimeError("StaticFrame.capture: the input buffers hold no rays yet; call step(rays_o, rays_d, ...) or fill frame.rays_o / frame.rays_d first")
        was = L.KERNEL_TIMER.enabled
        L.KERNEL_TIMER.enabled = False
        import gc
        gc.collect()
        try:
            side = torch.cuda.Stream(device=self.device)
            side.wait_stream(torch.cuda.current_stream())
            with torch.cuda.stream(side):
                for _ in range(2):
                    self._run()
            torch.cuda.current_stream().wait_stream(side)
            torch.cuda.synchronize()
            g = torch.cuda.CUDAGraph()
            self._occ_captured = self.model.accel.occ.occ_grid
            with torch.cuda.graph(g, stream=side):
                self.rendered, self.buffers, self.loss = self._run()
            self.graph = g
            self.captures += 1
        finally:
            L.KERNEL_TIMER.enabled = was
        return self

    def step(self, rays_o, rays_d, rays_h_appear=None):
        self.rays_o.copy_(rays_o, non_blocking=True)
        self.rays_d.copy_(rays_d, non_blocking=True)
        if self.h_appear is not None and rays_h_appear is not None:
            self.h_appear.copy_(rays_h_appear, non_blocking=True)
        cv = getattr(self.model, "ctrl_var", None)
        if cv is not None and hasattr(cv, "mix_weight"):
            if getattr(cv, "_w_dev", None) is None:
                cv._w_dev = torch.zeros((), device=self.device)
            cv._w_dev.fill_(cv.mix_weight())
        if self.graph is None and (self.use_graph or self.march_cap is None):
            self.capture()
        if self.graph is not None:
            occ = self.model.accel.occ.occ_grid
            if self._occ_captured is not None and occ.data_ptr() != self._occ_captured.data_ptr():
                self._occ_captured.copy_(occ)
            self.graph.replay()
        else:
            self.rendered, self.buffers, self.loss = self._run()
        return self.loss

    def counts(self):
        c = self.cnt.tolist()
        return {k: c[v] for k, v in CNT_SLOTS.items()}

    def check(self, retry=True):
        if int(self.cnt[CNT_SLOTS["overflow"]]) == 0:
            return True
        self.march_cap = self.kept_cap = None
        self._size(grow=1.25)
        self.graph = None
        if self.use_graph:
            self.capture()
        if retry:
            if self.graph is not None:
                self.graph.replay()
            else:
                self.rendered, self.buffers, self.loss = self._run()
        return False

    def volume_buffer(self):
        return sliced_volume_buffer(self.buffers, self.cnt)
```

Before: 24.39.

## Recompute color MLP activations in backward instead of storing four tiles

The forward kernel no longer writes the Z, Y1 and Y2 activation tiles to global memory. It keeps only the input tile X, and the backward kernels recompute the radiance-MLP hidden layers from X with extra tensor-core MMAs. The forward also drops the shared-memory fp32 accumulator staging: MMA fragments are written straight to f16 smem tiles, which frees smem so the kernel can declare three CTAs per SM. This cuts activation memory traffic to a quarter, at the cost of extra recompute in backward and slightly different rounding of the gradient values passed through f16.

```diff
diff --git a/neuralsim_b200/csrc/color_tc.cu b/neuralsim_b200/csrc/color_tc.cu
--- a/neuralsim_b200/csrc/color_tc.cu
+++ b/neuralsim_b200/csrc/color_tc.cu
@@ -68,28 +68,9 @@
 
 constexpr int kColorBwdCtasPerSM = 2;
 
-__global__ void __launch_bounds__(kTile)
-k_color_fwd(const PLMeta m, const __half *__restrict__ grid, const ColorNetDev net, const PointSrc ps, const float *__restrict__ view_dirs,
-            const float *__restrict__ h_appear, int64_t n, int max_level, float *__restrict__ sdf_out, float *__restrict__ nab_out,
-            float *__restrict__ rgb_out, float *__restrict__ x_out, uint8_t *__restrict__ Zt, uint8_t *__restrict__ Xt,
-            uint8_t *__restrict__ Y1t, uint8_t *__restrict__ Y2t, const OccCollect oc, const int64_t *__restrict__ n_dev) {
-    n = eff_n(n, n_dev);
-    extern __shared__ uint8_t dyn_smem[];
-    uint8_t *tiles = reinterpret_cast<uint8_t *>((reinterpret_cast<uintptr_t>(dyn_smem) + 1023) & ~uintptr_t(1023));
-    uint8_t *sX = tiles;
-    uint8_t *sU = sX + kTileBytes;
-    uint8_t *sW1 = sU + kTileBytes;
-    uint8_t *sW1T = sW1 + HW * NF * 2;
-    uint8_t *sR1 = sW1T + HW * NF * 2;
-    uint8_t *sR2 = sR1 + XW * XW * 2;
-    constexpr int kS = tc::acc_stride(64);
-    float *acc = reinterpret_cast<float *>(sR2 + XW * XW * 2);
-    __shared__ float sb1[HW], sW2[HW], srb1[XW], srb2[XW], sR3[3][XW];
-    __shared__ float sb2, srb3[3];
-
-    const int tid = threadIdx.x;
-    stage_W1(net.dec, sW1, tid);
-    stage_W1T(net.dec, sW1T, tid);
+constexpr int kColorFwdCtasPerSM = 3;
+
+__device__ __forceinline__ void stage_R1_R2(const ColorNetDev &net, uint8_t *sR1, uint8_t *sR2, int tid) {
     for (int e = tid; e < XW * XW; e += kTile) {
         const int j = e % XW, k = e / XW;
         const int rc = ref_col(k, net.n_appear);
@@ -98,13 +79,53 @@
         *reinterpret_cast<__half *>(sR1 + (k / 8) * (XW * 16) + j * 16 + (k % 8) * 2) = v1;
         *reinterpret_cast<__half *>(sR2 + (k / 8) * (XW * 16) + j * 16 + (k % 8) * 2) = v2;
     }
-    stage_decoder_vectors(net.dec, sb1, sW2, &sb2, tid);
+}
+
+__device__ __forceinline__ void stage_radiance_vectors(const ColorNetDev &net, float *srb1, float *srb2, float (*sR3)[XW], int tid) {
     if (tid < XW) {
         srb1[tid] = tid < net.rw ? __half2float(net.rb1[tid]) : 0.f;
         srb2[tid] = tid < net.rw ? __half2float(net.rb2[tid]) : 0.f;
 #pragma unroll
         for (int k = 0; k < 3; ++k) sR3[k][tid] = tid < net.rw ? __half2float(net.R3[k * net.rw + tid]) : 0.f;
     }
+}
+
+__device__ __forceinline__ void relu_bias_to_tile(const float (&y)[2][XW / 2], const float *bias, uint8_t *tile) {
+#pragma unroll
+    for (int h = 0; h < 2; ++h)
+#pragma unroll
+        for (int c = 0; c < XW / 8; ++c)
+#pragma unroll
+            for (int r = 0; r < 2; ++r) {
+                const int col = tc::frag_col(c);
+                tc::st_pair_f16(tile, tc::pair_off<kTile>(h * 64 + tc::frag_row(r), col), fmaxf(r16(y[h][4 * c + 2 * r] + bias[col]), 0.f),
+                                fmaxf(r16(y[h][4 * c + 2 * r + 1] + bias[col + 1]), 0.f));
+            }
+}
+
+__global__ void __launch_bounds__(kTile, kColorFwdCtasPerSM)
+k_color_fwd(const PLMeta m, const __half *__restrict__ grid, const ColorNetDev net, const PointSrc ps, const float *__restrict__ view_dirs,
+            const float *__restrict__ h_appear, int64_t n, int max_level, float *__restrict__ sdf_out, float *__restrict__ nab_out,
+            float *__restrict__ rgb_out, float *__restrict__ x_out, uint8_t *__restrict__ Xt, const OccCollect oc, const int64_t *__restrict__ n_dev) {
+    n = eff_n(n, n_dev);
+    extern __shared__ uint8_t dyn_smem[];
+    uint8_t *tiles = reinterpret_cast<uint8_t *>((reinterpret_cast<uintptr_t>(dyn_smem) + 1023) & ~uintptr_t(1023));
+    uint8_t *sX = tiles;
+    uint8_t *sU = sX + kTileBytes;
+    uint8_t *sS = sU + kTileBytes;
+    uint8_t *sW1 = sS + kTileBytes;
+    uint8_t *sW1T = sW1 + HW * NF * 2;
+    uint8_t *sR1 = sW1T + HW * NF * 2;
+    uint8_t *sR2 = sR1 + XW * XW * 2;
+    __shared__ float sb1[HW], sW2[HW], srb1[XW], srb2[XW], sR3[3][XW];
+    __shared__ float sb2, srb3[3];
+
+    const int tid = threadIdx.x;
+    stage_W1(net.dec, sW1, tid);
+    stage_W1T(net.dec, sW1T, tid);
+    stage_R1_R2(net, sR1, sR2, tid);
+    stage_decoder_vectors(net.dec, sb1, sW2, &sb2, tid);
+    stage_radiance_vectors(net, srb1, srb2, sR3, tid);
     if (tid == 0) {
         for (int k = 0; k < 3; ++k) srb3[k] = __half2float(net.rb3[k]);
     }
@@ -124,42 +145,64 @@
         gather_row_to_tile<kTile, kColorGatherU>(m, grid, xs, max_level, sX, tid);
         tc::fence_async_smem();
         __syncthreads();
-        tc::mma_to_rows<64, 0, 0, NF / 16>(acc, kS, 0, tc::kmajor(x_addr, kTile), tc::kmajor(w1_addr, HW), false);
+        {
+            float z[2][HW / 2];
+            tc::mma_m128<HW, 0, 0, NF / 16>(z, tc::kmajor(x_addr, kTile), tc::kmajor(w1_addr, HW), false);
+#pragma unroll
+            for (int h = 0; h < 2; ++h)
+#pragma unroll
+                for (int c = 0; c < HW / 8; ++c)
+#pragma unroll
+                    for (int r = 0; r < 2; ++r) {
+                        const int col = tc::frag_col(c);
+                        const uint32_t off = tc::pair_off<kTile>(h * 64 + tc::frag_row(r), col);
+                        float a[2], uu[2];
+#pragma unroll
+                        for (int j = 0; j < 2; ++j) {
+                            float s;
+                            softplus_as(r16(z[h][4 * c + 2 * r + j] + sb1[col + j]), spk, a[j], s);
+                            uu[j] = sW2[col + j] * s;
+                        }
+                        tc::st_pair_f16(sU, off, uu[0], uu[1]);
+                        tc::st_pair_f16(sS, off, a[0], a[1]);
+                    }
+        }
+        tc::fence_async_smem();
         __syncthreads();
         float out = 0.f;
-        uint8_t *zt = Zt ? Zt + tile * kTileBytes : nullptr;
 #pragma unroll 1
         for (int c = 0; c < HW / 8; ++c) {
-            float z[8], uu[8];
-            tc::acc_ld8(acc, kS, tid, c * 8, z);
-#pragma unroll
-            for (int j = 0; j < 8; ++j) {
-                z[j] = r16(z[j] + sb1[c * 8 + j]);
-                float a, s;
-                softplus_as(z[j], spk, a, s);
-                out = fmaf(r16(a), sW2[c * 8 + j], out);
-                uu[j] = sW2[c * 8 + j] * s;
-            }
-            *reinterpret_cast<uint4 *>(sU + c * kChunk + tid * 16) = tc::pack8_f16(uu);
-            if (zt) *reinterpret_cast<uint4 *>(zt + c * kChunk + tid * 16) = tc::pack8_f16(z);
+            float a8[8];
+            unpack8(*reinterpret_cast<const uint4 *>(sS + c * kChunk + tid * 16), a8);
+#pragma unroll
+            for (int j = 0; j < 8; ++j) out = fmaf(a8[j], sW2[c * 8 + j], out);
         }
         const float sdf = r16(out + sb2);
-        tc::fence_async_smem();
-        __syncthreads();
-        tc::mma_to_rows<32, 0, 0, HW / 16>(acc, kS, 0, tc::kmajor(u_addr, kTile), tc::kmajor(w1t_addr, NF), false);
+        {
+            float g[2][NF / 2];
+            tc::mma_m128<NF, 0, 0, HW / 16>(g, tc::kmajor(u_addr, kTile), tc::kmajor(w1t_addr, NF), false);
+#pragma unroll
+            for (int h = 0; h < 2; ++h)
+#pragma unroll
+                for (int c = 0; c < NF / 8; ++c)
+#pragma unroll
+                    for (int r = 0; r < 2; ++r)
+                        tc::st_pair_f16(sX + 4 * kChunk, tc::pair_off<kTile>(h * 64 + tc::frag_row(r), tc::frag_col(c)), g[h][4 * c + 2 * r],
+                                        g[h][4 * c + 2 * r + 1]);
+        }
         __syncthreads();
         float nacc[3] = {0.f, 0.f, 0.f};
 #pragma unroll 1
         for (uint32_t g4 = 0; g4 < 4; ++g4) {
             float gg[8];
-            tc::acc_ld8(acc, kS, tid, g4 * 8, gg);
+            unpack8(*reinterpret_cast<const uint4 *>(sX + (4 + g4) * kChunk + tid * 16), gg);
 #pragma unroll
             for (uint32_t q = 0; q < 4; ++q) {
                 const uint32_t p = g4 * 4 + q;
                 if ((int)m.level[p] <= max_level) {
                     float J0[3], J1[3];
                     level_jacobian(m, p, xs, grid, J0, J1);
-                    const float g0 = r16(gg[2 * q]), g1 = r16(gg[2 * q + 1]);
+                    const float g0 = gg[2 * q], g1 = gg[2 * q + 1];
 #pragma unroll
                     for (int d = 0; d < 3; ++d) nacc[d] = __fmaf_rn(g0, J0[d], nacc[d]);
 #pragma unroll
@@ -201,36 +244,28 @@
         }
         tc::fence_async_smem();
         __syncthreads();
-        tc::mma_to_rows<64, 0, 0, XW / 16>(acc, kS, 0, tc::kmajor(x_addr, kTile), tc::kmajor(r1_addr, XW), false);
-        __syncthreads();
-        uint8_t *y1t = Y1t ? Y1t + tile * kTileBytes : nullptr;
+        {
+            float y[2][XW / 2];
+            tc::mma_m128<XW, 0, 0, XW / 16>(y, tc::kmajor(x_addr, kTile), tc::kmajor(r1_addr, XW), false);
+            relu_bias_to_tile(y, srb1, sU);
+        }
+        tc::fence_async_smem();
+        __syncthreads();
+        {
+            float y[2][XW / 2];
+            tc::mma_m128<XW, 0, 0, XW / 16>(y, tc::kmajor(u_addr, kTile), tc::kmajor(r2_addr, XW), false);
+            relu_bias_to_tile(y, srb2, sS);
+        }
+        __syncthreads();
+        float o3[3] = {0.f, 0.f, 0.f};
 #pragma unroll 1
         for (int c = 0; c < XW / 8; ++c) {
             float y[8];
-            tc::acc_ld8(acc, kS, tid, c * 8, y);
-#pragma unroll
-            for (int j = 0; j < 8; ++j) y[j] = fmaxf(r16(y[j] + srb1[c * 8 + j]), 0.f);
-            const uint4 q = tc::pack8_f16(y);
-            *reinterpret_cast<uint4 *>(sU + c * kChunk + tid * 16) = q;
-            if (y1t) *reinterpret_cast<uint4 *>(y1t + c * kChunk + tid * 16) = q;
-        }
-        tc::fence_async_smem();
-        __syncthreads();
-        tc::mma_to_rows<64, 0, 0, XW / 16>(acc, kS, 0, tc::kmajor(u_addr, kTile), tc::kmajor(r2_addr, XW), false);
-        __syncthreads();
-        float o3[3] = {0.f, 0.f, 0.f};
-        uint8_t *y2t = Y2t ? Y2t + tile * kTileBytes : nullptr;
-#pragma unroll 1
-        for (int c = 0; c < XW / 8; ++c) {
-            float y[8];
-            tc::acc_ld8(acc, kS, tid, c * 8, y);
-#pragma unroll
-            for (int j = 0; j < 8; ++j) {
-                y[j] = fmaxf(r16(y[j] + srb2[c * 8 + j]), 0.f);
+            unpack8(*reinterpret_cast<const uint4 *>(sS + c * kChunk + tid * 16), y);
+#pragma unroll
+            for (int j = 0; j < 8; ++j)
 #pragma unroll
                 for (int k = 0; k < 3; ++k) o3[k] = fmaf(y[j], sR3[k][c * 8 + j], o3[k]);
-            }
-            if (y2t) *reinterpret_cast<uint4 *>(y2t + c * kChunk + tid * 16) = tc::pack8_f16(y);
         }
         if (valid) {
             sdf_out[i] = sdf;
@@ -243,14 +278,12 @@
                 if (x_out) x_out[i * 3 + d] = xn[d];
             }
         }
-        __syncthreads();
     }
 }
 
 __global__ void __launch_bounds__(kTile, kColorBwdCtasPerSM)
-k_color_rad_bwd(const ColorNetDev net, const uint8_t *__restrict__ Xt, const uint8_t *__restrict__ Y1t, const uint8_t *__restrict__ Y2t,
-                const float *__restrict__ rgb, const float *__restrict__ g_rgb, int64_t n, float *__restrict__ dh_out,
-                float *__restrict__ dR1, float *__restrict__ drb1, float *__restrict__ dR2, float *__restrict__ drb2,
+k_color_rad_bwd(const ColorNetDev net, const uint8_t *__restrict__ Xt, const float *__restrict__ rgb, const float *__restrict__ g_rgb, int64_t n,
+                float *__restrict__ dh_out, float *__restrict__ dR1, float *__restrict__ drb1, float *__restrict__ dR2, float *__restrict__ drb2,
                 float *__restrict__ dR3, float *__restrict__ drb3, const int64_t *__restrict__ n_dev) {
     n = eff_n(n, n_dev);
     constexpr int NE = 80;
@@ -259,27 +292,15 @@
     uint8_t *sT = tiles;
     uint8_t *sY1 = sT + 3 * kTileBytes;
     uint8_t *sXe = sY1 + kTile * NE * 2;
-    uint8_t *sR2T = sXe + kTile * NE * 2;
-    uint8_t *sR1h = sR2T + XW * XW * 2;
-    __shared__ float sR3[3][XW];
+    uint8_t *sR1 = sXe + kTile * NE * 2;
+    uint8_t *sR2 = sR1 + XW * XW * 2;
+    __shared__ float srb1[XW], srb2[XW], sR3[3][XW], sgy[3][kTile];
     __shared__ float sdb3[3];
     __shared__ __align__(8) uint64_t mbar_ld;
 
     const int tid = threadIdx.x, lane = tid & 31;
-    for (int e = tid; e < XW * XW; e += kTile) {
-        const int i = e % XW, j = e / XW;
-        const __half v = (j < net.rw && i < net.rw) ? net.R2[j * net.rw + i] : __float2half_rn(0.f);
-        *reinterpret_cast<__half *>(sR2T + (j / 8) * (XW * 16) + i * 16 + (j % 8) * 2) = v;
-    }
-    for (int e = tid; e < NF * XW; e += kTile) {
-        const int k = e % NF, j = e / NF;
-        const __half v = j < net.rw ? net.R1[j * net.rin + 22 + k] : __float2half_rn(0.f);
-        *reinterpret_cast<__half *>(sR1h + (j / 8) * (NF * 16) + k * 16 + (j % 8) * 2) = v;
-    }
-    if (tid < XW) {
-#pragma unroll
-        for (int k = 0; k < 3; ++k) sR3[k][tid] = tid < net.rw ? __half2float(net.R3[k * net.rw + tid]) : 0.f;
-    }
+    stage_R1_R2(net, sR1, sR2, tid);
+    stage_radiance_vectors(net, srb1, srb2, sR3, tid);
     *reinterpret_cast<uint4 *>(sY1 + 8 * kChunk + tid * 16) = make_uint4(0x00003C00u, 0, 0, 0);
     *reinterpret_cast<uint4 *>(sY1 + 9 * kChunk + tid * 16) = make_uint4(0, 0, 0, 0);
     *reinterpret_cast<uint4 *>(sXe + 9 * kChunk + tid * 16) = make_uint4(0, 0, 0, 0);
@@ -296,23 +317,19 @@
     tc::fence_async_smem();
     __syncthreads();
     const uint32_t t_addr = tc::smem_u32(sT), y1_addr = tc::smem_u32(sY1), xe_addr = tc::smem_u32(sXe);
-    const uint32_t r2t_addr = tc::smem_u32(sR2T), r1h_addr = tc::smem_u32(sR1h);
+    const uint32_t r1_addr = tc::smem_u32(sR1), r2_addr = tc::smem_u32(sR2);
     uint32_t ld_phase = 0;
     bool first_tile = true;
 
     const int64_t n_tiles = (n + kTile - 1) / kTile;
     auto fetch = [&](int64_t tile) {
-        tc::mbar_arrive_expect_tx(&mbar_ld, 3 * kTileBytes);
-        tc::tma_load_bulk(sT + 2 * kTileBytes, Y2t + tile * kTileBytes, kTileBytes, &mbar_ld);
-        tc::tma_load_bulk(sY1, Y1t + tile * kTileBytes, kTileBytes, &mbar_ld);
+        tc::mbar_arrive_expect_tx(&mbar_ld, kTileBytes);
         tc::tma_load_bulk(sXe, Xt + tile * kTileBytes, kTileBytes, &mbar_ld);
     };
     if (tid == 0 && (int64_t)blockIdx.x < n_tiles) fetch(blockIdx.x);
     for (int64_t tile = blockIdx.x; tile < n_tiles; tile += gridDim.x) {
         const int64_t i = tile * kTile + tid;
         const bool valid = i < n;
-        tc::mbar_wait(&mbar_ld, ld_phase);
-        ld_phase ^= 1;
         float gy[3] = {0.f, 0.f, 0.f};
         if (valid && g_rgb) {
 #pragma unroll
@@ -327,25 +344,49 @@
         }
 #pragma unroll
         for (int k = 0; k < 3; ++k) {
-            const float sgy = warp_sum(gy[k]);
-            if (lane == 0 && sgy != 0.f) atomicAdd(&sdb3[k], sgy);
-        }
-#pragma unroll 1
-        for (int c = 0; c < 8; ++c) {
-            float y2[8], d[8];
-            unpack8(*reinterpret_cast<const uint4 *>(sT + 2 * kTileBytes + c * kChunk + tid * 16), y2);
-#pragma unroll
-            for (int j = 0; j < 8; ++j) {
-                const float v = gy[0] * sR3[0][c * 8 + j] + gy[1] * sR3[1][c * 8 + j] + gy[2] * sR3[2][c * 8 + j];
-                d[j] = y2[j] > 0.f ? v : 0.f;
-            }
-            *reinterpret_cast<uint4 *>(sT + c * kChunk + tid * 16) = tc::pack8_f16(d);
+            sgy[k][tid] = gy[k];
+            const float sgy_sum = warp_sum(gy[k]);
+            if (lane == 0 && sgy_sum != 0.f) atomicAdd(&sdb3[k], sgy_sum);
+        }
+        tc::mbar_wait(&mbar_ld, ld_phase);
+        ld_phase ^= 1;
+        {
+            float y[2][XW / 2];
+            tc::mma_m128<XW, 0, 0, XW / 16>(y, tc::kmajor(xe_addr, kTile), tc::kmajor(r1_addr, XW), false);
+            relu_bias_to_tile(y, srb1, sY1);
+        }
+        tc::fence_async_smem();
+        __syncthreads();
+        {
+            float y[2][XW / 2];
+            tc::mma_m128<XW, 0, 0, XW / 16>(y, tc::kmajor(y1_addr, kTile), tc::kmajor(r2_addr, XW), false);
+#pragma unroll
+            for (int h = 0; h < 2; ++h)
+#pragma unroll
+                for (int r = 0; r < 2; ++r) {
+                    const int row = h * 64 + tc::frag_row(r);
+                    const float g0 = sgy[0][row], g1 = sgy[1][row], g2 = sgy[2][row];
+#pragma unroll
+                    for (int c = 0; c < XW / 8; ++c) {
+                        const int col = tc::frag_col(c);
+                        const uint32_t off = tc::pair_off<kTile>(row, col);
+                        float y2[2], d[2];
+#pragma unroll
+                        for (int j = 0; j < 2; ++j) {
+                            y2[j] = fmaxf(r16(y[h][4 * c + 2 * r + j] + srb2[col + j]), 0.f);
+                            const float v = g0 * sR3[0][col + j] + g1 * sR3[1][col + j] + g2 * sR3[2][col + j];
+                            d[j] = y2[j] > 0.f ? v : 0.f;
+                        }
+                        tc::st_pair_f16(sT + 2 * kTileBytes, off, y2[0], y2[1]);
+                        tc::st_pair_f16(sT, off, d[0], d[1]);
+                    }
+                }
         }
         tc::fence_async_smem();
         __syncthreads();
         {
             float dy[2][XW / 2];
-            tc::mma_m128<64, 0, 0, XW / 16>(dy, tc::kmajor(t_addr, kTile), tc::kmajor(r2t_addr, XW), false);
+            tc::mma_m128<64, 0, 1, XW / 16>(dy, tc::kmajor(t_addr, kTile), tc::mnmajor(r2_addr, XW), false);
 #pragma unroll
             for (int h = 0; h < 2; ++h)
 #pragma unroll
@@ -360,7 +401,7 @@
         tc::fence_async_smem();
         __syncthreads();
         float dh[2][NF / 2];
-        tc::mma_m128<32, 0, 0, XW / 16>(dh, tc::kmajor(t_addr + kTileBytes, kTile), tc::kmajor(r1h_addr, NF), false);
+        tc::mma_m128<32, 0, 1, XW / 16>(dh, tc::kmajor(t_addr + kTileBytes, kTile), tc::mnmajor(r1_addr, XW), false);
         tc::mma_m64<NE, 1, 1, kTile / 16>(xa, tc::mnmajor(t_addr, kTile), tc::mnmajor(y1_addr, kTile), true);
         tc::mma_m64<NE, 1, 1, kTile / 16>(xb, tc::mnmajor(t_addr + kTileBytes, kTile), tc::mnmajor(xe_addr, kTile), true);
         tc::mma_m64<8, 1, 1, kTile / 16>(x3, tc::mnmajor(t_addr + 2 * kTileBytes, kTile), tc::mnmajor(xe_addr + 8 * kChunk, kTile), true);
@@ -413,7 +454,7 @@
 }
 
 __global__ void __launch_bounds__(kTile, kColorBwdCtasPerSM)
-k_color_sdf_bwd(const PLMeta m, const __half *__restrict__ grid, const ColorNetDev net, const PointSrc ps, const uint8_t *__restrict__ Zt,
+k_color_sdf_bwd(const PLMeta m, const __half *__restrict__ grid, const ColorNetDev net, const PointSrc ps,
                 const uint8_t *__restrict__ Xt, const float *__restrict__ g_nab, const float *__restrict__ g_sdf, const float *__restrict__ dh_r,
                 int64_t n, int max_level, float *__restrict__ d_grid, float *__restrict__ d_W1, float *__restrict__ d_b1, float *__restrict__ d_W2,
                 float *__restrict__ d_b2, const int64_t *__restrict__ n_dev) {
@@ -430,14 +471,14 @@
     constexpr int kS = tc::acc_stride(2 * NF);
     float *stage = reinterpret_cast<float *>(sT);
     static_assert(kTile * kS * 4 <= 3 * kTileBytes, "the staged rows must fit in T");
-    __shared__ float sW2[HW], sdsdf[kTile];
+    __shared__ float sb1[HW], sW2[HW], sdsdf[kTile];
     __shared__ float sdb2;
     __shared__ __align__(8) uint64_t mbar_ld;
 
     const int tid = threadIdx.x, lane = tid & 31;
     stage_W1(net.dec, sW1, tid);
     stage_W1T(net.dec, sW1T, tid);
-    stage_decoder_vectors(net.dec, nullptr, sW2, nullptr, tid);
+    stage_decoder_vectors(net.dec, sb1, sW2, nullptr, tid);
     *reinterpret_cast<uint4 *>(sHe + 4 * kChunk + tid * 16) = make_uint4(0x00003C00u, 0, 0, 0);
     *reinterpret_cast<uint4 *>(sGe + 4 * kChunk + tid * 16) = make_uint4(0x00003C00u, 0, 0, 0);
     *reinterpret_cast<uint4 *>(sHe + 5 * kChunk + tid * 16) = make_uint4(0, 0, 0, 0);
@@ -462,8 +503,7 @@
 
     const int64_t n_tiles = (n + kTile - 1) / kTile;
     auto fetch = [&](int64_t tile) {
-        tc::mbar_arrive_expect_tx(&mbar_ld, kTileBytes + 4 * kChunk);
-        tc::tma_load_bulk(sZ, Zt + tile * kTileBytes, kTileBytes, &mbar_ld);
+        tc::mbar_arrive_expect_tx(&mbar_ld, 4 * kChunk);
         tc::tma_load_bulk(sHe, Xt + tile * kTileBytes, 4 * kChunk, &mbar_ld);
     };
     if (tid == 0 && (int64_t)blockIdx.x < n_tiles) fetch(blockIdx.x);
@@ -480,20 +520,6 @@
         }
         const float dsdf = (valid && g_sdf) ? g_sdf[i] : 0.f;
         sdsdf[tid] = dsdf;
-        tc::mbar_wait(&mbar_ld, ld_phase);
-        ld_phase ^= 1;
-#pragma unroll 1
-        for (int c = 0; c < 8; ++c) {
-            float z[8], uu[8];
-            unpack8(*reinterpret_cast<const uint4 *>(sZ + c * kChunk + tid * 16), z);
-#pragma unroll
-            for (int j = 0; j < 8; ++j) {
-                float a, s;
-                softplus_as(z[j], spk, a, s);
-                uu[j] = sW2[c * 8 + j] * s;
-            }
-            *reinterpret_cast<uint4 *>(sT + kTileBytes + c * kChunk + tid * 16) = tc::pack8_f16(uu);
-        }
 #pragma unroll 4
         for (uint32_t p = 0; p < 16; ++p) {
             uint32_t packed = 0;
@@ -507,6 +533,31 @@
                 packed = *reinterpret_cast<const uint32_t *>(&h);
             }
             *reinterpret_cast<uint32_t *>(sGe + (p >> 2) * kChunk + tid * 16 + (p & 3) * 4) = packed;
+        }
+        tc::mbar_wait(&mbar_ld, ld_phase);
+        ld_phase ^= 1;
+        {
+            float z[2][HW / 2];
+            tc::mma_m128<HW, 0, 0, NF / 16>(z, tc::kmajor(he_addr, kTile), tc::kmajor(w1_addr, HW), false);
+#pragma unroll
+            for (int h = 0; h < 2; ++h)
+#pragma unroll
+                for (int c = 0; c < HW / 8; ++c)
+#pragma unroll
+                    for (int r = 0; r < 2; ++r) {
+                        const int col = tc::frag_col(c);
+                        const uint32_t off = tc::pair_off<kTile>(h * 64 + tc::frag_row(r), col);
+                        float zz[2], uu[2];
+#pragma unroll
+                        for (int j = 0; j < 2; ++j) {
+                            float a, s;
+                            zz[j] = r16(z[h][4 * c + 2 * r + j] + sb1[col + j]);
+                            softplus_as(zz[j], spk, a, s);
+                            uu[j] = sW2[col + j] * s;
+                        }
+                        tc::st_pair_f16(sZ, off, zz[0], zz[1]);
+                        tc::st_pair_f16(sT + kTileBytes, off, uu[0], uu[1]);
+                    }
         }
         tc::fence_async_smem();
         __syncthreads();
@@ -655,18 +706,19 @@
     if (n == 0) return 0;
     NSB_REQUIRE(meta && params_half && net && sdf && nablas && rgb && view_dirs, "nsb_fused_color_fwd: NULL argument");
     NSB_REQUIRE(x || (rays_o && rays_d && t), "nsb_fused_color_fwd: need x or (rays_o, rays_d, t)");
-    NSB_REQUIRE((act_z && act_x && act_y1 && act_y2) || (!act_z && !act_x && !act_y1 && !act_y2), "nsb_fused_color_fwd: pass all four activation buffers or none");
+    NSB_REQUIRE(act_x || (!act_z && !act_y1 && !act_y2), "nsb_fused_color_fwd: act_x is the activation buffer kept for the backward; pass it or none");
+    (void)act_z, (void)act_y1, (void)act_y2;
     PLMeta m;
     ColorNetDev d;
     if (int rc = make_net(net, meta, &m, &d, "nsb_fused_color_fwd")) return rc;
     NSB_REQUIRE(d.n_appear == 0 || h_appear, "nsb_fused_color_fwd: h_appear is NULL but the net has %d appearance channels", d.n_appear);
-    constexpr int kSmem = 2 * kTileBytes + 2 * HW * NF * 2 + 2 * XW * XW * 2 + kTile * tc::acc_stride(64) * 4 + 1024;
+    constexpr int kSmem = 3 * kTileBytes + 2 * HW * NF * 2 + 2 * XW * XW * 2 + 1024;
     opt_in_smem(k_color_fwd, kSmem);
+    if (int rc = require_ctas_per_sm(k_color_fwd, kTile, kSmem, kColorFwdCtasPerSM, "nsb_fused_color_fwd")) return rc;
     const PointSrc ps{x, rays_o, rays_d, t, ridx};
-    k_color_fwd<<<persistent_grid(n_tiles(n), 2), kTile, kSmem, (cudaStream_t)stream>>>(m, (const __half *)params_half, d, ps, view_dirs, h_appear, n,
-                                                                                        max_level < 0 ? -1 : max_level, sdf, nablas, rgb, x_out, (uint8_t *)act_z,
-                                                                                        (uint8_t *)act_x, (uint8_t *)act_y1, (uint8_t *)act_y2,
-                                                                                        occ_collect_of(collect), dn.a);
+    k_color_fwd<<<persistent_grid(n_tiles(n), kColorFwdCtasPerSM), kTile, kSmem, (cudaStream_t)stream>>>(
+        m, (const __half *)params_half, d, ps, view_dirs, h_appear, n, max_level < 0 ? -1 : max_level, sdf, nablas, rgb, x_out, (uint8_t *)act_x,
+        occ_collect_of(collect), dn.a);
     return check_launch("nsb_fused_color_fwd");
 }
 
@@ -678,7 +730,8 @@
                                    void *stream) {
     const DevCounts dn = take_counts();
     if (n == 0) return 0;
-    NSB_REQUIRE(meta && params_half && net && act_z && act_x && act_y1 && act_y2 && rgb && dh_scratch, "nsb_fused_color_bwd: NULL argument");
+    NSB_REQUIRE(meta && params_half && net && act_x && rgb && dh_scratch, "nsb_fused_color_bwd: NULL argument");
+    (void)act_z, (void)act_y1, (void)act_y2;
     NSB_REQUIRE(d_grid && d_W1 && d_b1 && d_W2 && d_b2 && d_R1 && d_rb1 && d_R2 && d_rb2 && d_R3 && d_rb3, "nsb_fused_color_bwd: NULL gradient buffer");
     NSB_REQUIRE(x || (rays_o && rays_d && t), "nsb_fused_color_bwd: need x or (rays_o, rays_d, t)");
     PLMeta m;
@@ -687,12 +740,11 @@
     cudaStream_t s = (cudaStream_t)stream;
     const float *dh = nullptr;
     if (g_rgb) {
-        constexpr int kSmemR = 3 * kTileBytes + 2 * kTile * 80 * 2 + XW * XW * 2 + NF * XW * 2 + 1024;
+        constexpr int kSmemR = 3 * kTileBytes + 2 * kTile * 80 * 2 + 2 * XW * XW * 2 + 1024;
         opt_in_smem(k_color_rad_bwd, kSmemR);
         if (int rc = require_ctas_per_sm(k_color_rad_bwd, kTile, kSmemR, kColorBwdCtasPerSM, "nsb_fused_color_bwd(radiance)")) return rc;
-        k_color_rad_bwd<<<persistent_grid(n_tiles(n), kColorBwdCtasPerSM), kTile, kSmemR, s>>>(d, (const uint8_t *)act_x, (const uint8_t *)act_y1,
-                                                                                               (const uint8_t *)act_y2, rgb, g_rgb, n, dh_scratch, d_R1,
-                                                                                               d_rb1, d_R2, d_rb2, d_R3, d_rb3, dn.a);
+        k_color_rad_bwd<<<persistent_grid(n_tiles(n), kColorBwdCtasPerSM), kTile, kSmemR, s>>>(d, (const uint8_t *)act_x, rgb, g_rgb, n, dh_scratch,
+                                                                                               d_R1, d_rb1, d_R2, d_rb2, d_R3, d_rb3, dn.a);
         if (int rc = check_launch("nsb_fused_color_bwd(radiance)")) return rc;
         dh = dh_scratch;
     }
@@ -700,7 +752,7 @@
     opt_in_smem(k_color_sdf_bwd, kSmemS);
     if (int rc = require_ctas_per_sm(k_color_sdf_bwd, kTile, kSmemS, kColorBwdCtasPerSM, "nsb_fused_color_bwd(sdf)")) return rc;
     const PointSrc ps{x, rays_o, rays_d, t, ridx};
-    k_color_sdf_bwd<<<persistent_grid(n_tiles(n), kColorBwdCtasPerSM), kTile, kSmemS, s>>>(m, (const __half *)params_half, d, ps, (const uint8_t *)act_z, (const uint8_t *)act_x,
+    k_color_sdf_bwd<<<persistent_grid(n_tiles(n), kColorBwdCtasPerSM), kTile, kSmemS, s>>>(m, (const __half *)params_half, d, ps, (const uint8_t *)act_x,
                                                                           g_nablas, g_sdf, dh, n, max_level < 0 ? -1 : max_level, d_grid, d_W1, d_b1, d_W2, d_b2, dn.a);
     return check_launch("nsb_fused_color_bwd(sdf)");
 }
diff --git a/neuralsim_b200/csrc/tc_util.cuh b/neuralsim_b200/csrc/tc_util.cuh
--- a/neuralsim_b200/csrc/tc_util.cuh
+++ b/neuralsim_b200/csrc/tc_util.cuh
@@ -150,35 +150,6 @@
                 *reinterpret_cast<float2 *>(acc + row * stride + col) = make_float2(d[h][4 * c + 2 * i], d[h][4 * c + 2 * i + 1]);
             }
 }
-template <int N>
-__device__ __forceinline__ void frag_load(float (&d)[2][N / 2], const float *acc, int stride, int col0) {
-    const int w = threadIdx.x >> 5, l = threadIdx.x & 31;
-#pragma unroll
-    for (int h = 0; h < 2; ++h)
-#pragma unroll
-        for (int c = 0; c < N / 8; ++c)
-#pragma unroll
-            for (int i = 0; i < 2; ++i) {
-                const int row = h * 64 + w * 16 + (l >> 2) + 8 * i, col = col0 + c * 8 + 2 * (l & 3);
-                const float2 v = *reinterpret_cast<const float2 *>(acc + row * stride + col);
-                d[h][4 * c + 2 * i] = v.x;
-                d[h][4 * c + 2 * i + 1] = v.y;
-            }
-}
-template <int N, int TA, int TB, int KSTEPS>
-__device__ __forceinline__ void mma_to_rows(float *acc, int stride, int col0, const Operand &a, const Operand &b, bool accumulate) {
-    float d[2][N / 2];
-    if (accumulate) frag_load<N>(d, acc, stride, col0);
-    else {
-#pragma unroll
-        for (int h = 0; h < 2; ++h)
-#pragma unroll
-            for (int i = 0; i < N / 2; ++i) d[h][i] = 0.f;
-    }
-    mma_m128<N, TA, TB, KSTEPS>(d, a, b, accumulate);
-    frag_store<N>(d, acc, stride, col0);
-}
-
 __device__ __forceinline__ void acc_ld8(const float *acc, int stride, int row, int col, float (&v)[8]) {
     const float4 a = *reinterpret_cast<const float4 *>(acc + row * stride + col), b = *reinterpret_cast<const float4 *>(acc + row * stride + col + 4);
     v[0] = a.x; v[1] = a.y; v[2] = a.z; v[3] = a.w; v[4] = b.x; v[5] = b.y; v[6] = b.z; v[7] = b.w;
diff --git a/neuralsim_b200/fields/fused_color.py b/neuralsim_b200/fields/fused_color.py
--- a/neuralsim_b200/fields/fused_color.py
+++ b/neuralsim_b200/fields/fused_color.py
@@ -21,8 +21,8 @@
         x = torch.empty(n, 3, dtype=torch.float32, device=dev)
         acts = None
         if keep:
-            acts = torch.empty(4, int(L.lib().nsb_color_tile_bytes(L.c_i64(n))), dtype=torch.uint8, device=dev)
-        ap = [L.ptr(acts[k]) if keep else None for k in range(4)]
+            acts = torch.empty(int(L.lib().nsb_color_tile_bytes(L.c_i64(n))), dtype=torch.uint8, device=dev)
+        ap = [None, L.ptr(acts) if keep else None, None, None]
         with L.KERNEL_TIMER.time("fused_color_fwd", n):
             L.check(L.lib().nsb_fused_color_fwd(meta.c_ref, L.ptr(grid16, "f16"), ctypes.byref(net), None, L.ptr(rays_o, "f32"), L.ptr(rays_d, "f32"),
                                                 L.ptr(ridx, "i64"), L.ptr(t, "f32"), L.ptr(view_dirs, "f32"), L.ptr(h_appear, "f32", allow_none=True),
@@ -58,8 +58,8 @@
         dh = torch.empty(n, 32, dtype=torch.float32, device=dev)
         with L.KERNEL_TIMER.time("fused_color_bwd", n):
             L.check(L.lib().nsb_fused_color_bwd(meta.c_ref, L.ptr(grid16, "f16"), ctypes.byref(net), None, L.ptr(rays_o, "f32"), L.ptr(rays_d, "f32"),
-                                                L.ptr(ridx, "i64"), L.ptr(t, "f32"), L.c_i64(n), L.c_i32(ctx.max_level), L.ptr(acts[0]), L.ptr(acts[1]),
-                                                L.ptr(acts[2]), L.ptr(acts[3]), L.ptr(rgb), L.ptr(g_sdf, allow_none=True), L.ptr(g_nab, allow_none=True),
+                                                L.ptr(ridx, "i64"), L.ptr(t, "f32"), L.c_i64(n), L.c_i32(ctx.max_level), None, L.ptr(acts), None, None,
+                                                L.ptr(rgb), L.ptr(g_sdf, allow_none=True), L.ptr(g_nab, allow_none=True),
                                                 L.ptr(g_rgb, allow_none=True), L.ptr(dh), *[L.ptr(g) for g in grads], L.stream_ptr()),
                     "fused_color_bwd")
         return (None,) * 7 + tuple(grads)
diff --git a/neuralsim_b200/graphics/neus_static.py b/neuralsim_b200/graphics/neus_static.py
--- a/neuralsim_b200/graphics/neus_static.py
+++ b/neuralsim_b200/graphics/neus_static.py
@@ -159,8 +159,8 @@
         nab = torch.empty(n, 3, dtype=torch.float32, device=dev)
         rgb = torch.empty(n, 3, dtype=torch.float32, device=dev)
         x = torch.empty(n, 3, dtype=torch.float32, device=dev)
-        acts = torch.empty(4, int(L.lib().nsb_color_tile_bytes(L.c_i64(n))), dtype=torch.uint8, device=dev) if keep_acts else None
-        ap = [L.ptr(acts[k]) if keep_acts else None for k in range(4)]
+        acts = torch.empty(int(L.lib().nsb_color_tile_bytes(L.c_i64(n))), dtype=torch.uint8, device=dev) if keep_acts else None
+        ap = [None, L.ptr(acts) if keep_acts else None, None, None]
         P = L.ptr
         with L.KERNEL_TIMER.time("fused_color_fwd", n):
             _call(L.lib().nsb_fused_color_fwd, "fused_color_fwd", st.cnt, CNT_SLOTS["kept"], None,
@@ -196,7 +196,7 @@
         with L.KERNEL_TIMER.time("fused_color_bwd", n):
             _call(L.lib().nsb_fused_color_bwd, "fused_color_bwd", st.cnt, CNT_SLOTS["kept"], None,
                   st.meta.c_ref, P(st.grid16, "f16"), ctypes.byref(st.net), None, P(st.rays_o, "f32"), P(st.rays_d, "f32"), P(ctx.ridx, "i64"),
-                  P(ctx.t, "f32"), L.c_i64(n), L.c_i32(st.ml), P(acts[0]), P(acts[1]), P(acts[2]), P(acts[3]), P(rgb), P(g_sdf, allow_none=True),
+                  P(ctx.t, "f32"), L.c_i64(n), L.c_i32(st.ml), None, P(acts), None, None, P(rgb), P(g_sdf, allow_none=True),
                   P(g_nab, allow_none=True), P(g_rgb, allow_none=True), P(dh), *[P(g) for g in grads], L.stream_ptr())
         return (None,) * 6 + tuple(grads)
 
```

Result: no change. 24.74 (median of 6 runs) (+1.5%).
